# MarkJhonBao/InfantPoseEstimation_GaussianBias

Measured on AMD Instinct MI355X. Metric: images/sec (train fwd+bwd) HRFormer-S 256x192, higher is better.
Workload: dtype bf16; 1 GPU; HRFormer-small + fusion head, 256x192 -> 64x48, K=17, train step fwd+bwd+AdamW, DropPath 0.1, BN train; global_batch=64, per_gpu_batch=64, parallelism=dp1, launch=hipGraph replay, branches on concurrent HIP streams

## Files before the change

### infantposeestimation_gaussianbias_amd/csrc/pk_block.hip

```cpp
#include "pk_common.h"

typedef __attribute__((ext_vector_type(8))) short bf16x8;
typedef __attribute__((ext_vector_type(4))) float f32x4;
typedef __attribute__((ext_vector_type(4))) short s16x4;
typedef __attribute__((ext_vector_type(4))) unsigned int u32x4;
typedef __attribute__((ext_vector_type(2))) unsigned int u32x2;

#define OOB_OFF 0x80000000u
#define MAKE_RSRC(ptr) __builtin_amdgcn_make_buffer_rsrc(const_cast<uint16_t*>(ptr), 0, 0x7ffffff0, 0x00020000)
#define LOG2E_F 1.44269504088896340736f
#define MFMA(a, b, c) __builtin_amdgcn_mfma_f32_16x16x32_bf16(a, b, c, 0, 0, 0)
#define MFMA16(a, b, c) __builtin_amdgcn_mfma_f32_16x16x16bf16_1k(a, b, c, 0, 0, 0)
#define LO4(v) __builtin_shufflevector(v, v, 0, 1, 2, 3)
#define HI4(v) __builtin_shufflevector(v, v, 4, 5, 6, 7)
#define LDS_FENCE() asm volatile("s_waitcnt lgkmcnt(0)" ::: "memory")

struct MlpArgs {
    const uint16_t* x;
    const uint16_t* dy;
    uint16_t* out;
    const float *gamma, *beta, *b1, *b2;
    const float* scale;
    const uint16_t* w1;
    const uint16_t* w2;
    const uint16_t* w1t;
    const uint16_t* w2t;
    float* part;
    int M, rows_per_sample;
    float eps;
};

__device__ __forceinline__ int hid(int t, int i) { return 32 * (t >> 1) + 8 * (i >> 2) + 4 * (t & 1) + (i & 3); }
__device__ __forceinline__ float blo(uint32_t u) { return __uint_as_float(u << 16); }
__device__ __forceinline__ float bhi(uint32_t u) { return __uint_as_float(u & 0xffff0000u); }
__device__ __forceinline__ bf16x8 pack2(const f32x4 a, const f32x4 b) {
    const u32x4 v = {pack_bf16x2(a[0], a[1]), pack_bf16x2(a[2], a[3]), pack_bf16x2(b[0], b[1]), pack_bf16x2(b[2], b[3])};
    return __builtin_bit_cast(bf16x8, v);
}
__device__ __forceinline__ f32x4 unpack4(const u32x2 v) { return (f32x4){blo(v[0]), bhi(v[0]), blo(v[1]), bhi(v[1])}; }
__device__ __forceinline__ u32x2 pack4(const f32x4 v) { return (u32x2){pack_bf16x2(v[0], v[1]), pack_bf16x2(v[2], v[3])}; }
__device__ __forceinline__ float sum8(const bf16x8 f) {
    const u32x4 v = __builtin_bit_cast(u32x4, f);
    return ((blo(v[0]) + bhi(v[0])) + (blo(v[1]) + bhi(v[1]))) + ((blo(v[2]) + bhi(v[2])) + (blo(v[3]) + bhi(v[3])));
}
__device__ __forceinline__ bf16x8 tr_frag32(const uint16_t* tile, int pitch, int col0, int lane) {
    const int g = lane >> 4, i = lane & 15;
    const uint16_t* a0 = tile + (4 * g + (i >> 2)) * pitch + col0 + 4 * (i & 3);
    const s16x4 lo = __builtin_amdgcn_ds_read_tr16_b64_v4i16((__attribute__((address_space(3))) s16x4*)a0);
    const s16x4 hi = __builtin_amdgcn_ds_read_tr16_b64_v4i16((__attribute__((address_space(3))) s16x4*)(a0 + 16 * pitch));
    return (bf16x8){lo[0], lo[1], lo[2], lo[3], hi[0], hi[1], hi[2], hi[3]};
}

template <typename RowFn, typename K0Fn>
__device__ __forceinline__ void stage_frags(u32x4* dst, const uint16_t* __restrict__ src, int nfrag, int ld, RowFn row, K0Fn k0) {
    for (int idx = threadIdx.x; idx < nfrag * 64; idx += blockDim.x) {
        const int f = idx >> 6, l = idx & 63;
        dst[idx] = *reinterpret_cast<const u32x4*>(src + (size_t)row(f, l & 15) * ld + k0(f) + 8 * (l >> 4));
    }
}
#define LDS_FRAG(base, f, lane) __builtin_bit_cast(bf16x8, (base)[(f) * 64 + (lane)])
template <bool OPAQUE>
__device__ __forceinline__ int opaque_lane(int lane) {
    if (OPAQUE) asm volatile("" : "+v"(lane));
    return lane;
}

template <int NK>
__device__ __forceinline__ void ln_row(const u32x4 (&xr)[NK], const float (&gam)[NK][8], const float (&bet)[NK][8], float inv_c, float eps,
                                       bf16x8 (&vf)[NK], float& mean, float& rstd) {
    float v[NK][8];
    float s = 0.f;
#pragma unroll
    for (int k = 0; k < NK; ++k)
#pragma unroll
        for (int j = 0; j < 4; ++j) {
            v[k][2 * j] = blo(xr[k][j]);
            v[k][2 * j + 1] = bhi(xr[k][j]);
            s += v[k][2 * j] + v[k][2 * j + 1];
        }
    s = xor16_sum(s);
    s = xor32_sum(s);
    mean = s * inv_c;
    float q = 0.f;
#pragma unroll
    for (int k = 0; k < NK; ++k)
#pragma unroll
        for (int j = 0; j < 8; ++j) {
            v[k][j] -= mean;
            q += v[k][j] * v[k][j];
        }
    q = xor16_sum(q);
    q = xor32_sum(q);
    rstd = rsqrtf(q * inv_c + eps);
#pragma unroll
    for (int k = 0; k < NK; ++k) {
        u32x4 o;
#pragma unroll
        for (int j = 0; j < 4; ++j)
            o[j] = pack_bf16x2(v[k][2 * j] * rstd * gam[k][2 * j] + bet[k][2 * j], v[k][2 * j + 1] * rstd * gam[k][2 * j + 1] + bet[k][2 * j + 1]);
        vf[k] = __builtin_bit_cast(bf16x8, o);
    }
}
template <int NK>
__device__ __forceinline__ void scale_rows(const u32x4 (&r)[NK], float sc, bf16x8 (&f)[NK]) {
#pragma unroll
    for (int k = 0; k < NK; ++k) {
        u32x4 o;
#pragma unroll
        for (int j = 0; j < 4; ++j) o[j] = pack_bf16x2(blo(r[k][j]) * sc, bhi(r[k][j]) * sc);
        f[k] = __builtin_bit_cast(bf16x8, o);
    }
}

template <int C>
__global__ void __launch_bounds__(256) k_mlp_fwd(MlpArgs p) {
    constexpr int HD = 4 * C, NK = C / 32, NT = HD / 16, NS = HD / 32, NCT = C / 16, RT = 2;
    __shared__ __attribute__((aligned(16))) u32x4 sW1[NT * NK * 64];
    __shared__ __attribute__((aligned(16))) u32x4 sW2[NCT * NS * 64];
    __shared__ __attribute__((aligned(16))) float sB1[HD];
    const int tid = threadIdx.x, lane_ = tid & 63, wave = tid >> 6, i16 = lane_ & 15, g = lane_ >> 4;
    stage_frags(sW1, p.w1, NT * NK, C, [](int f, int i) { return hid(f / NK, i); }, [](int f) { return 32 * (f % NK); });
    stage_frags(sW2, p.w2, NCT * NS, HD, [](int f, int i) { return 16 * (f / NS) + i; }, [](int f) { return 32 * (f % NS); });
    for (int i = tid; i < HD; i += 256) sB1[i] = p.b1[i];
    float gam[NK][8], bet[NK][8];
#pragma unroll
    for (int k = 0; k < NK; ++k)
#pragma unroll
        for (int j = 0; j < 8; ++j) {
            gam[k][j] = p.gamma[32 * k + 8 * g + j];
            bet[k][j] = p.beta[32 * k + 8 * g + j];
        }
    f32x4 b2v[NCT];
#pragma unroll
    for (int ct = 0; ct < NCT; ++ct) b2v[ct] = *reinterpret_cast<const f32x4*>(p.b2 + 16 * ct + 4 * g);
    __syncthreads();
    const auto rx = MAKE_RSRC(p.x);
    const auto ro = MAKE_RSRC(p.out);
    const int ngroups = (p.M + 16 * RT - 1) / (16 * RT);
    const float inv_c = 1.f / (float)C;
    const f32x4 zero = {0.f, 0.f, 0.f, 0.f};
    for (int grp = blockIdx.x * 4 + wave; grp < ngroups; grp += gridDim.x * 4) {
        const int lane = opaque_lane<C != 32>(lane_);
        u32x4 xr[RT][NK];
        u32x2 xo[RT][NCT];
        unsigned rbase[RT];
        float sc[RT];
#pragma unroll
        for (int rt = 0; rt < RT; ++rt) {
            const int row = grp * 16 * RT + 16 * rt + i16;
            const bool ok = row < p.M;
            rbase[rt] = ok ? (unsigned)row * (unsigned)(C * 2) : OOB_OFF;
#pragma unroll
            for (int k = 0; k < NK; ++k) xr[rt][k] = __builtin_amdgcn_raw_buffer_load_b128(rx, ok ? rbase[rt] + (32 * k + 8 * g) * 2 : OOB_OFF, 0, 0);
#pragma unroll
            for (int ct = 0; ct < NCT; ++ct) xo[rt][ct] = __builtin_amdgcn_raw_buffer_load_b64(rx, ok ? rbase[rt] + (16 * ct + 4 * g) * 2 : OOB_OFF, 0, 0);
            sc[rt] = (p.scale && ok) ? p.scale[row / p.rows_per_sample] : 1.f;
        }
        bf16x8 vf[RT][NK];
#pragma unroll
        for (int rt = 0; rt < RT; ++rt) {
            float mean, rstd;
            ln_row<NK>(xr[rt], gam, bet, inv_c, p.eps, vf[rt], mean, rstd);
        }
        f32x4 y[RT][NCT];
#pragma unroll
        for (int rt = 0; rt < RT; ++rt)
#pragma unroll
            for (int ct = 0; ct < NCT; ++ct) y[rt][ct] = zero;
#pragma unroll
        for (int s = 0; s < NS; ++s) {
            f32x4 h[RT][2];
#pragma unroll
            for (int u = 0; u < 2; ++u) {
                const int t = 2 * s + u;
                const f32x4 bias = *reinterpret_cast<const f32x4*>(&sB1[32 * s + 8 * g + 4 * u]);
#pragma unroll
                for (int rt = 0; rt < RT; ++rt) h[rt][u] = bias;
#pragma unroll
                for (int k = 0; k < NK; ++k) {
                    const bf16x8 a = LDS_FRAG(sW1, t * NK + k, lane);
#pragma unroll
                    for (int rt = 0; rt < RT; ++rt) h[rt][u] = MFMA(a, vf[rt][k], h[rt][u]);
                }
#pragma unroll
                for (int rt = 0; rt < RT; ++rt) h[rt][u] = gelu_erf(h[rt][u]);
            }
            bf16x8 hf[RT];
#pragma unroll
            for (int rt = 0; rt < RT; ++rt) hf[rt] = pack2(h[rt][0], h[rt][1]);
#pragma unroll
            for (int ct = 0; ct < NCT; ++ct) {
                const bf16x8 a = LDS_FRAG(sW2, ct * NS + s, lane);
#pragma unroll
                for (int rt = 0; rt < RT; ++rt) y[rt][ct] = MFMA(a, hf[rt], y[rt][ct]);
            }
        }
#pragma unroll
        for (int rt = 0; rt < RT; ++rt)
#pragma unroll
            for (int ct = 0; ct < NCT; ++ct) {
                const f32x4 o = (y[rt][ct] + b2v[ct]) * sc[rt] + unpack4(xo[rt][ct]);
                __builtin_amdgcn_raw_buffer_store_b64(pack4(o), ro, rbase[rt] == OOB_OFF ? OOB_OFF : rbase[rt] + (16 * ct + 4 * g) * 2, 0, 0);
            }
    }
}

template <int NK, int NCT, int WAVES, bool RESIDENT>
__global__ void __launch_bounds__(64 * WAVES) k_mlp_fwd_w(MlpArgs p, int C, int c_real, int HD) {
    constexpr int RT = 2, NF = 2 * NK + NCT, NLD = (NF + WAVES - 1) / WAVES;
    extern __shared__ __attribute__((aligned(16))) unsigned char smem_w[];
    const int NS = HD >> 5, n_slots = RESIDENT ? NS : 2;
    u32x4* ring = reinterpret_cast<u32x4*>(smem_w);
    float* sB1 = reinterpret_cast<float*>(smem_w + n_slots * NF * 1024);
    const int tid = threadIdx.x, lane = tid & 63, wave = tid >> 6, i16 = lane & 15, g = lane >> 4;
    const auto rw1 = MAKE_RSRC(p.w1), rw2 = MAKE_RSRC(p.w2);
    unsigned soff[NLD], sstep[NLD];
#pragma unroll
    for (int j = 0; j < NLD; ++j) {
        const int f = wave + WAVES * j;
        if (f < 2 * NK) {
            const int u = f / NK, k = f - u * NK, col = 32 * k + 8 * g;
            soff[j] = col < C ? (unsigned)((hid(u, i16) * C + col) * 2) : OOB_OFF;
            sstep[j] = 64u * (unsigned)C;
        } else if (f < NF) {
            const int ct = f - 2 * NK;
            soff[j] = (unsigned)(((16 * ct + i16) * HD + 8 * g) * 2);
            sstep[j] = 64u;
        } else {
            soff[j] = OOB_OFF;
            sstep[j] = 0u;
        }
    }
    u32x4 st[NLD];
    auto load_slice = [&](int s) {
#pragma unroll
        for (int j = 0; j < NLD; ++j) {
            const int f = wave + WAVES * j;
            st[j] = f < 2 * NK ? __builtin_amdgcn_raw_buffer_load_b128(rw1, soff[j] + sstep[j] * (unsigned)s, 0, 0)
                               : __builtin_amdgcn_raw_buffer_load_b128(rw2, soff[j] + sstep[j] * (unsigned)s, 0, 0);
        }
    };
    auto write_slice = [&](int slot) {
#pragma unroll
        for (int j = 0; j < NLD; ++j) {
            const int f = wave + WAVES * j;
            if (f < NF) ring[(slot * NF + f) * 64 + lane] = st[j];
        }
    };
    load_slice(0);
    for (int i = tid; i < HD; i += 64 * WAVES) sB1[i] = p.b1[i];
    if (RESIDENT) {
        for (int s = 0; s < NS; ++s) {
            write_slice(s);
            if (s + 1 < NS) load_slice(s + 1);
        }
        __syncthreads();
    }
    const auto rx = MAKE_RSRC(p.x);
    const auto ro = MAKE_RSRC(p.out);
    const auto rgam = __builtin_amdgcn_make_buffer_rsrc(const_cast<float*>(p.gamma), 0, C * 4, 0x00020000);
    const auto rbet = __builtin_amdgcn_make_buffer_rsrc(const_cast<float*>(p.beta), 0, C * 4, 0x00020000);
    const auto rb2 = __builtin_amdgcn_make_buffer_rsrc(const_cast<float*>(p.b2), 0, C * 4, 0x00020000);
    const float inv_c = 1.f / (float)c_real, n_pad = (float)(32 * NK - c_real);
    const f32x4 zero = {0.f, 0.f, 0.f, 0.f};
    const int ngroups = (p.M + 16 * RT - 1) / (16 * RT);
    auto process = [&](const int grp) {
        unsigned rbase[RT];
        float sc[RT];
        bf16x8 vf[RT][NK];
#pragma unroll
        for (int rt = 0; rt < RT; ++rt) {
            const int row = grp * 16 * RT + 16 * rt + i16;
            const bool ok = row < p.M;
            rbase[rt] = ok ? (unsigned)row * (unsigned)(C * 2) : OOB_OFF;
            sc[rt] = (p.scale && ok) ? p.scale[row / p.rows_per_sample] : 1.f;
            u32x4 xr[NK];
#pragma unroll
            for (int k = 0; k < NK; ++k) xr[k] = __builtin_amdgcn_raw_buffer_load_b128(rx, (ok && 32 * k + 8 * g < C) ? rbase[rt] + (32 * k + 8 * g) * 2 : OOB_OFF, 0, 0);
            float v[NK][8];
            float sm = 0.f;
#pragma unroll
            for (int k = 0; k < NK; ++k)
#pragma unroll
                for (int j = 0; j < 4; ++j) {
                    v[k][2 * j] = blo(xr[k][j]);
                    v[k][2 * j + 1] = bhi(xr[k][j]);
                    sm += v[k][2 * j] + v[k][2 * j + 1];
                }
            sm = xor16_sum(sm);
            sm = xor32_sum(sm);
            const float mean = sm * inv_c;
            float q = 0.f;
#pragma unroll
            for (int k = 0; k < NK; ++k)
#pragma unroll
                for (int j = 0; j < 8; ++j) {
                    v[k][j] -= mean;
                    q += v[k][j] * v[k][j];
                }
            q = xor16_sum(q);
            q = xor32_sum(q);
            const float rstd = rsqrtf(fmaxf(q - n_pad * mean * mean, 0.f) * inv_c + p.eps);
#pragma unroll
            for (int k = 0; k < NK; ++k) {
                const f32x4 g0 = __builtin_bit_cast(f32x4, __builtin_amdgcn_raw_buffer_load_b128(rgam, (32 * k + 8 * g) * 4, 0, 0));
                const f32x4 g1 = __builtin_bit_cast(f32x4, __builtin_amdgcn_raw_buffer_load_b128(rgam, (32 * k + 8 * g + 4) * 4, 0, 0));
                const f32x4 b0 = __builtin_bit_cast(f32x4, __builtin_amdgcn_raw_buffer_load_b128(rbet, (32 * k + 8 * g) * 4, 0, 0));
                const f32x4 b1 = __builtin_bit_cast(f32x4, __builtin_amdgcn_raw_buffer_load_b128(rbet, (32 * k + 8 * g + 4) * 4, 0, 0));
                u32x4 o;
                o[0] = pack_bf16x2(v[k][0] * rstd * g0[0] + b0[0], v[k][1] * rstd * g0[1] + b0[1]);
                o[1] = pack_bf16x2(v[k][2] * rstd * g0[2] + b0[2], v[k][3] * rstd * g0[3] + b0[3]);
                o[2] = pack_bf16x2(v[k][4] * rstd * g1[0] + b1[0], v[k][5] * rstd * g1[1] + b1[1]);
                o[3] = pack_bf16x2(v[k][6] * rstd * g1[2] + b1[2], v[k][7] * rstd * g1[3] + b1[3]);
                vf[rt][k] = __builtin_bit_cast(bf16x8, o);
            }
        }
        if (!RESIDENT) {
            write_slice(0);
            if (NS > 1) load_slice(1);
        }
        f32x4 y[RT][NCT];
#pragma unroll
        for (int rt = 0; rt < RT; ++rt)
#pragma unroll
            for (int ct = 0; ct < NCT; ++ct) y[rt][ct] = zero;
#pragma unroll 1
        for (int s = 0; s < NS; ++s) {
            if (!RESIDENT) {
                __syncthreads();
                if (s + 1 < NS) write_slice((s + 1) & 1);
                if (s + 2 < NS) load_slice(s + 2);
            }
            const u32x4* fr = ring + (RESIDENT ? s : (s & 1)) * NF * 64;
            f32x4 h[RT][2];
#pragma unroll
            for (int u = 0; u < 2; ++u) {
                const f32x4 bias = *reinterpret_cast<const f32x4*>(&sB1[32 * s + 8 * g + 4 * u]);
#pragma unroll
                for (int rt = 0; rt < RT; ++rt) h[rt][u] = bias;
            }
#pragma unroll
            for (int k = 0; k < NK; ++k)
#pragma unroll
                for (int u = 0; u < 2; ++u) {
                    const bf16x8 a = LDS_FRAG(fr, u * NK + k, lane);
#pragma unroll
                    for (int rt = 0; rt < RT; ++rt) h[rt][u] = MFMA(a, vf[rt][k], h[rt][u]);
                }
            bf16x8 hf[RT];
#pragma unroll
            for (int rt = 0; rt < RT; ++rt) {
                hf[rt] = pack2(gelu_erf_poly(h[rt][0]), gelu_erf_poly(h[rt][1]));
            }
#pragma unroll
            for (int ct = 0; ct < NCT; ++ct) {
                const bf16x8 a = LDS_FRAG(fr, 2 * NK + ct, lane);
#pragma unroll
                for (int rt = 0; rt < RT; ++rt) y[rt][ct] = MFMA(a, hf[rt], y[rt][ct]);
            }
        }
#pragma unroll
        for (int rt = 0; rt < RT; ++rt)
#pragma unroll
            for (int ct = 0; ct < NCT; ++ct) {
                const unsigned off = rbase[rt] == OOB_OFF ? OOB_OFF : rbase[rt] + (16 * ct + 4 * g) * 2;
                const u32x2 xo = __builtin_amdgcn_raw_buffer_load_b64(rx, off, 0, 0);
                const f32x4 b2v = __builtin_bit_cast(f32x4, __builtin_amdgcn_raw_buffer_load_b128(rb2, (16 * ct + 4 * g) * 4, 0, 0));
                const f32x4 o = (y[rt][ct] + b2v) * sc[rt] + unpack4(xo);
                __builtin_amdgcn_raw_buffer_store_b64(pack4(o), ro, off, 0, 0);
            }
    };
    if (RESIDENT) {
        for (int grp = blockIdx.x * WAVES + wave; grp < ngroups; grp += gridDim.x * WAVES) process(grp);
    } else {
        process(blockIdx.x * WAVES + wave);
    }
}

template <int C>
__global__ void __launch_bounds__(256) k_mlp_bwd_dx(MlpArgs p) {
    constexpr int HD = 4 * C, NK = C / 32, NT = HD / 16, NS = HD / 32, NCT = C / 16, RT = 2;
    __shared__ __attribute__((aligned(16))) u32x4 sW1[NT * NK * 64];
    __shared__ __attribute__((aligned(16))) u32x4 sW2T[NT * NK * 64];
    __shared__ __attribute__((aligned(16))) u32x4 sW1T[NCT * NS * 64];
    __shared__ __attribute__((aligned(16))) float sB1[HD];
    __shared__ float sRed[4][2][C];
    const int tid = threadIdx.x, lane_ = tid & 63, wave = tid >> 6, i16 = lane_ & 15, g = lane_ >> 4;
    stage_frags(sW1, p.w1, NT * NK, C, [](int f, int i) { return hid(f / NK, i); }, [](int f) { return 32 * (f % NK); });
    stage_frags(sW2T, p.w2t, NT * NK, C, [](int f, int i) { return hid(f / NK, i); }, [](int f) { return 32 * (f % NK); });
    stage_frags(sW1T, p.w1t, NCT * NS, HD, [](int f, int i) { return 16 * (f / NS) + i; }, [](int f) { return 32 * (f % NS); });
    for (int i = tid; i < HD; i += 256) sB1[i] = p.b1[i];
    float gam[NK][8], bet[NK][8];
#pragma unroll
    for (int k = 0; k < NK; ++k)
#pragma unroll
        for (int j = 0; j < 8; ++j) {
            gam[k][j] = p.gamma[32 * k + 8 * g + j];
            bet[k][j] = p.beta[32 * k + 8 * g + j];
        }
    f32x4 gamA[NCT], dgam[NCT], dbet[NCT];
    const f32x4 zero = {0.f, 0.f, 0.f, 0.f};
#pragma unroll
    for (int ct = 0; ct < NCT; ++ct) {
        gamA[ct] = *reinterpret_cast<const f32x4*>(p.gamma + 16 * ct + 4 * g);
        dgam[ct] = dbet[ct] = zero;
    }
    __syncthreads();
    const auto rx = MAKE_RSRC(p.x);
    const auto rg = MAKE_RSRC(p.dy);
    const auto ro = MAKE_RSRC(p.out);
    const int ngroups = (p.M + 16 * RT - 1) / (16 * RT);
    const float inv_c = 1.f / (float)C;
    for (int grp = blockIdx.x * 4 + wave; grp < ngroups; grp += gridDim.x * 4) {
        const int lane = opaque_lane<true>(lane_);
        u32x4 xr[RT][NK], dyr[RT][NK];
        u32x2 xo[RT][NCT], dyo[RT][NCT];
        unsigned rbase[RT];
        float sc[RT];
#pragma unroll
        for (int rt = 0; rt < RT; ++rt) {
            const int row = grp * 16 * RT + 16 * rt + i16;
            const bool ok = row < p.M;
            rbase[rt] = ok ? (unsigned)row * (unsigned)(C * 2) : OOB_OFF;
#pragma unroll
            for (int k = 0; k < NK; ++k) {
                const unsigned off = ok ? rbase[rt] + (32 * k + 8 * g) * 2 : OOB_OFF;
                xr[rt][k] = __builtin_amdgcn_raw_buffer_load_b128(rx, off, 0, 0);
                dyr[rt][k] = __builtin_amdgcn_raw_buffer_load_b128(rg, off, 0, 0);
            }
#pragma unroll
            for (int ct = 0; ct < NCT; ++ct) {
                const unsigned off = ok ? rbase[rt] + (16 * ct + 4 * g) * 2 : OOB_OFF;
                xo[rt][ct] = __builtin_amdgcn_raw_buffer_load_b64(rx, off, 0, 0);
                dyo[rt][ct] = __builtin_amdgcn_raw_buffer_load_b64(rg, off, 0, 0);
            }
            sc[rt] = (p.scale && ok) ? p.scale[row / p.rows_per_sample] : 1.f;
        }
        bf16x8 vf[RT][NK], gf[RT][NK];
        float mean[RT], rstd[RT];
#pragma unroll
        for (int rt = 0; rt < RT; ++rt) {
            ln_row<NK>(xr[rt], gam, bet, inv_c, p.eps, vf[rt], mean[rt], rstd[rt]);
            scale_rows<NK>(dyr[rt], sc[rt], gf[rt]);
        }
        f32x4 dv[RT][NCT];
#pragma unroll
        for (int rt = 0; rt < RT; ++rt)
#pragma unroll
            for (int ct = 0; ct < NCT; ++ct) dv[rt][ct] = zero;
#pragma unroll
        for (int s = 0; s < NS; ++s) {
            f32x4 dz[RT][2];
#pragma unroll
            for (int u = 0; u < 2; ++u) {
                const int t = 2 * s + u;
                const f32x4 bias = *reinterpret_cast<const f32x4*>(&sB1[32 * s + 8 * g + 4 * u]);
                f32x4 z[RT], dh[RT];
#pragma unroll
                for (int rt = 0; rt < RT; ++rt) {
                    z[rt] = bias;
                    dh[rt] = zero;
                }
#pragma unroll
                for (int k = 0; k < NK; ++k) {
                    const bf16x8 a1 = LDS_FRAG(sW1, t * NK + k, lane), a2 = LDS_FRAG(sW2T, t * NK + k, lane);
#pragma unroll
                    for (int rt = 0; rt < RT; ++rt) {
                        z[rt] = MFMA(a1, vf[rt][k], z[rt]);
                        dh[rt] = MFMA(a2, gf[rt][k], dh[rt]);
                    }
                }
#pragma unroll
                for (int rt = 0; rt < RT; ++rt) dz[rt][u] = dh[rt] * gelu_grad(z[rt]);
            }
            bf16x8 dzf[RT];
#pragma unroll
            for (int rt = 0; rt < RT; ++rt) dzf[rt] = pack2(dz[rt][0], dz[rt][1]);
#pragma unroll
            for (int ct = 0; ct < NCT; ++ct) {
                const bf16x8 a = LDS_FRAG(sW1T, ct * NS + s, lane);
#pragma unroll
                for (int rt = 0; rt < RT; ++rt) dv[rt][ct] = MFMA(a, dzf[rt], dv[rt][ct]);
            }
        }
#pragma unroll
        for (int rt = 0; rt < RT; ++rt) {
            f32x4 xh[NCT];
            float s1 = 0.f, s2 = 0.f;
#pragma unroll
            for (int ct = 0; ct < NCT; ++ct) {
                xh[ct] = (unpack4(xo[rt][ct]) - mean[rt]) * rstd[rt];
#pragma unroll
                for (int r = 0; r < 4; ++r) {
                    const float gh = dv[rt][ct][r] * gamA[ct][r];
                    s1 += gh;
                    s2 += gh * xh[ct][r];
                }
                dgam[ct] += dv[rt][ct] * xh[ct];
                dbet[ct] += dv[rt][ct];
            }
            s1 = xor16_sum(s1);
            s1 = xor32_sum(s1);
            s2 = xor16_sum(s2);
            s2 = xor32_sum(s2);
            const float m1 = s1 * inv_c, m2 = s2 * inv_c;
#pragma unroll
            for (int ct = 0; ct < NCT; ++ct) {
                const f32x4 o = (dv[rt][ct] * gamA[ct] - m1 - xh[ct] * m2) * rstd[rt] + unpack4(dyo[rt][ct]);
                __builtin_amdgcn_raw_buffer_store_b64(pack4(o), ro, rbase[rt] == OOB_OFF ? OOB_OFF : rbase[rt] + (16 * ct + 4 * g) * 2, 0, 0);
            }
        }
    }
#pragma unroll
    for (int ct = 0; ct < NCT; ++ct)
#pragma unroll
        for (int r = 0; r < 4; ++r) {
            float a = dgam[ct][r], b = dbet[ct][r];
            a = lanes_sum<16>(a);
            b = lanes_sum<16>(b);
            if (i16 == 0) {
                sRed[wave][0][16 * ct + 4 * g + r] = a;
                sRed[wave][1][16 * ct + 4 * g + r] = b;
            }
        }
    __syncthreads();
    if (tid < 2 * C) {
        const int which = tid / C, c = tid - which * C;
        p.part[(size_t)blockIdx.x * 2 * C + tid] = ((sRed[0][which][c] + sRed[1][which][c]) + sRed[2][which][c]) + sRed[3][which][c];
    }
}

template <int C, int HS>
__global__ void __launch_bounds__(256) k_mlp_bwd_dw(MlpArgs p) {
    constexpr int NK = C / 32, NTS = HS / 16, NSP = HS / 32, NCT = C / 16, RT = 2;
    constexpr int PV = C + 8, PH = 40;
    constexpr int TILE_HALFS = 2 * 32 * PV + 2 * 32 * PH;
    constexpr int SLAB = 2 * HS * C + HS + C;
    constexpr int SCRATCH_BYTES = (4 * TILE_HALFS * 2 > SLAB * 4) ? 4 * TILE_HALFS * 2 : SLAB * 4;
    __shared__ __attribute__((aligned(16))) u32x4 sW1[NTS * NK * 64];
    __shared__ __attribute__((aligned(16))) u32x4 sW2T[NTS * NK * 64];
    __shared__ __attribute__((aligned(16))) float sB1[HS];
    __shared__ __attribute__((aligned(16))) unsigned char sScratch[SCRATCH_BYTES];
    const int tid = threadIdx.x, lane_ = tid & 63, wave = tid >> 6, i16 = lane_ & 15, g = lane_ >> 4;
    const int h0 = blockIdx.y * HS;
    stage_frags(sW1, p.w1 + (size_t)h0 * C, NTS * NK, C, [](int f, int i) { return 16 * (f / NK) + i; }, [](int f) { return 32 * (f % NK); });
    stage_frags(sW2T, p.w2t + (size_t)h0 * C, NTS * NK, C, [](int f, int i) { return 16 * (f / NK) + i; }, [](int f) { return 32 * (f % NK); });
    for (int i = tid; i < HS; i += 256) sB1[i] = p.b1[h0 + i];
    uint16_t* tV = reinterpret_cast<uint16_t*>(sScratch) + wave * TILE_HALFS;
    uint16_t* tG = tV + 32 * PV;
    uint16_t* tH = tG + 32 * PV;
    uint16_t* tD = tH + 32 * PH;
    float gam[NK][8], bet[NK][8];
#pragma unroll
    for (int k = 0; k < NK; ++k)
#pragma unroll
        for (int j = 0; j < 8; ++j) {
            gam[k][j] = p.gamma[32 * k + 8 * g + j];
            bet[k][j] = p.beta[32 * k + 8 * g + j];
        }
    const f32x4 zero = {0.f, 0.f, 0.f, 0.f};
    f32x4 dW1[NTS][NCT], dW2[NCT][NTS];
    float db1[NTS], db2[NCT];
#pragma unroll
    for (int t = 0; t < NTS; ++t) {
        db1[t] = 0.f;
#pragma unroll
        for (int ct = 0; ct < NCT; ++ct) dW1[t][ct] = dW2[ct][t] = zero;
    }
#pragma unroll
    for (int ct = 0; ct < NCT; ++ct) db2[ct] = 0.f;
    __syncthreads();
    const auto rx = MAKE_RSRC(p.x);
    const auto rg = MAKE_RSRC(p.dy);
    const int ngroups = (p.M + 16 * RT - 1) / (16 * RT);
    const float inv_c = 1.f / (float)C;
    for (int grp = blockIdx.x * 4 + wave; grp < ngroups; grp += gridDim.x * 4) {
        const int lane = opaque_lane<true>(lane_);
        u32x4 xr[RT][NK], dyr[RT][NK];
        float sc[RT];
#pragma unroll
        for (int rt = 0; rt < RT; ++rt) {
            const int row = grp * 16 * RT + 16 * rt + i16;
            const bool ok = row < p.M;
#pragma unroll
            for (int k = 0; k < NK; ++k) {
                const unsigned off = ok ? (unsigned)row * (unsigned)(C * 2) + (32 * k + 8 * g) * 2 : OOB_OFF;
                xr[rt][k] = __builtin_amdgcn_raw_buffer_load_b128(rx, off, 0, 0);
                dyr[rt][k] = __builtin_amdgcn_raw_buffer_load_b128(rg, off, 0, 0);
            }
            sc[rt] = (p.scale && ok) ? p.scale[row / p.rows_per_sample] : 1.f;
        }
        bf16x8 vf[RT][NK], gf[RT][NK];
#pragma unroll
        for (int rt = 0; rt < RT; ++rt) {
            float mean, rstd;
            ln_row<NK>(xr[rt], gam, bet, inv_c, p.eps, vf[rt], mean, rstd);
            scale_rows<NK>(dyr[rt], sc[rt], gf[rt]);
#pragma unroll
            for (int k = 0; k < NK; ++k) {
                *reinterpret_cast<bf16x8*>(tV + (16 * rt + i16) * PV + 32 * k + 8 * g) = vf[rt][k];
                *reinterpret_cast<bf16x8*>(tG + (16 * rt + i16) * PV + 32 * k + 8 * g) = gf[rt][k];
            }
        }
        LDS_FENCE();
        bf16x8 vT[NCT], gT[NCT];
#pragma unroll
        for (int ct = 0; ct < NCT; ++ct) {
            vT[ct] = tr_frag32(tV, PV, 16 * ct, lane);
            gT[ct] = tr_frag32(tG, PV, 16 * ct, lane);
            db2[ct] += sum8(gT[ct]);
        }
#pragma unroll
        for (int sp = 0; sp < NSP; ++sp) {
#pragma unroll
            for (int u = 0; u < 2; ++u) {
                const int t = 2 * sp + u;
                const f32x4 bias = *reinterpret_cast<const f32x4*>(&sB1[16 * t + 4 * g]);
                f32x4 z[RT], dh[RT];
#pragma unroll
                for (int rt = 0; rt < RT; ++rt) {
                    z[rt] = bias;
                    dh[rt] = zero;
                }
#pragma unroll
                for (int k = 0; k < NK; ++k) {
                    const bf16x8 a1 = LDS_FRAG(sW1, t * NK + k, lane), a2 = LDS_FRAG(sW2T, t * NK + k, lane);
#pragma unroll
                    for (int rt = 0; rt < RT; ++rt) {
                        z[rt] = MFMA(a1, vf[rt][k], z[rt]);
                        dh[rt] = MFMA(a2, gf[rt][k], dh[rt]);
                    }
                }
#pragma unroll
                for (int rt = 0; rt < RT; ++rt) {
                    f32x4 hh, dz;
                    gelu_both(z[rt], hh, dz);
                    dz *= dh[rt];
                    *reinterpret_cast<u32x2*>(tH + (16 * rt + i16) * PH + 16 * u + 4 * g) = pack4(hh);
                    *reinterpret_cast<u32x2*>(tD + (16 * rt + i16) * PH + 16 * u + 4 * g) = pack4(dz);
                }
            }
            LDS_FENCE();
#pragma unroll
            for (int u = 0; u < 2; ++u) {
                const int t = 2 * sp + u;
                const bf16x8 hT = tr_frag32(tH, PH, 16 * u, lane), dT = tr_frag32(tD, PH, 16 * u, lane);
                db1[t] += sum8(dT);
#pragma unroll
                for (int ct = 0; ct < NCT; ++ct) {
                    dW2[ct][t] = MFMA(gT[ct], hT, dW2[ct][t]);
                    dW1[t][ct] = MFMA(dT, vT[ct], dW1[t][ct]);
                }
            }
            LDS_FENCE();
        }
    }
    float* slab = reinterpret_cast<float*>(sScratch);
#pragma unroll 1
    for (int w = 0; w < 4; ++w) {
        __syncthreads();
        if (wave == w) {
#pragma unroll
            for (int t = 0; t < NTS; ++t) {
#pragma unroll
                for (int ct = 0; ct < NCT; ++ct)
#pragma unroll
                    for (int r = 0; r < 4; ++r) {
                        float* a = slab + (16 * t + 4 * g + r) * C + 16 * ct + i16;
                        float* b = slab + HS * C + (16 * ct + 4 * g + r) * HS + 16 * t + i16;
                        *a = (w ? *a : 0.f) + dW1[t][ct][r];
                        *b = (w ? *b : 0.f) + dW2[ct][t][r];
                    }
                float v = db1[t];
                v = xor16_sum(v);
                v = xor32_sum(v);
                if (g == 0) {
                    float* a = slab + 2 * HS * C + 16 * t + i16;
                    *a = (w ? *a : 0.f) + v;
                }
            }
#pragma unroll
            for (int ct = 0; ct < NCT; ++ct) {
                float v = db2[ct];
                v = xor16_sum(v);
                v = xor32_sum(v);
                if (g == 0) {
                    float* a = slab + 2 * HS * C + HS + 16 * ct + i16;
                    *a = (w ? *a : 0.f) + v;
                }
            }
        }
    }
    __syncthreads();
    float* dst = p.part + ((size_t)blockIdx.y * gridDim.x + blockIdx.x) * SLAB;
    for (int i = tid * 4; i < SLAB; i += 1024) *reinterpret_cast<f32x4*>(dst + i) = *reinterpret_cast<const f32x4*>(slab + i);
}

struct AttnArgs {
    const uint16_t* x;
    const uint16_t* dy;
    uint16_t* out;
    const int32_t* rowmap;
    const float *gamma, *beta, *table, *bqkv, *bproj, *scale;
    const uint16_t *wqkv, *wproj;
    const uint16_t *wqkv_t, *wproj_t;
    uint16_t* o_save;
    float* lse;
    uint16_t* dqkv;
    uint16_t* u_save;
    float* part;
    int n_windows, windows_per_sample;
    float eps, softmax_scale;
};
#define AT_N 49
__device__ __forceinline__ int rel_a7(int t) { return 13 * (t / 7) + t % 7; }

template <int C>
__global__ void __launch_bounds__(256) k_attn_fwd(AttnArgs p) {
    constexpr int HEADS = C / 32, NK = C / 32, NCT = C / 16;
    __shared__ __attribute__((aligned(16))) u32x4 sWqkv[HEADS * 6 * NK * 64];
    __shared__ __attribute__((aligned(16))) u32x4 sWp[NCT * HEADS * 64];
    __shared__ __attribute__((aligned(16))) float sBqkv[3 * C];
    __shared__ float sBias[HEADS][176];
    const int tid = threadIdx.x, lane_ = tid & 63, wave = tid >> 6, g_ = lane_ >> 4;
    stage_frags(sWqkv, p.wqkv, HEADS * 6 * NK, C,
                [](int f, int i) {
                    const int k_ = f % NK, r = f / NK, et = r & 1, part = (r >> 1) % 3, h = r / 6;
                    (void)k_;
                    return part * C + 32 * h + (part == 2 ? hid(et, i) : 16 * et + i);
                },
                [](int f) { return 32 * (f % NK); });
    stage_frags(sWp, p.wproj, NCT * HEADS, C, [](int f, int i) { return 16 * (f / HEADS) + i; }, [](int f) { return 32 * (f % HEADS); });
    for (int i = tid; i < 3 * C; i += 256) sBqkv[i] = p.bqkv[i];
    for (int i = tid; i < HEADS * 169; i += 256) sBias[i / 169][i % 169] = p.table[(i % 169) * HEADS + i / 169];
    float gam[NK][8], bet[NK][8];
#pragma unroll
    for (int k = 0; k < NK; ++k)
#pragma unroll
        for (int j = 0; j < 8; ++j) {
            gam[k][j] = p.gamma[32 * k + 8 * g_ + j];
            bet[k][j] = p.beta[32 * k + 8 * g_ + j];
        }
    f32x4 bpv[NCT];
#pragma unroll
    for (int ct = 0; ct < NCT; ++ct) bpv[ct] = *reinterpret_cast<const f32x4*>(p.bproj + 16 * ct + 4 * g_);
    int aj[4][4];
#pragma unroll
    for (int cj = 0; cj < 4; ++cj)
#pragma unroll
        for (int r = 0; r < 4; ++r) {
            const int j = 16 * cj + 4 * g_ + r;
            aj[cj][r] = j < AT_N ? 84 - rel_a7(j) : -1;
        }
    __syncthreads();
    const auto rx = MAKE_RSRC(p.x);
    const auto ro = MAKE_RSRC(p.out);
    const float inv_c = 1.f / (float)C;
    const f32x4 zero = {0.f, 0.f, 0.f, 0.f};
    for (int w = blockIdx.x * 4 + wave; w < p.n_windows; w += gridDim.x * 4) {
        const int lane = opaque_lane<true>(lane_), i16 = lane & 15, g = lane >> 4;
        int row[4];
        u32x4 xr[4][NK];
        u32x2 xo[4][NCT];
#pragma unroll
        for (int t = 0; t < 4; ++t) {
            const int n = 16 * t + i16;
            row[t] = n < AT_N ? p.rowmap[w * AT_N + n] : -1;
        }
#pragma unroll
        for (int t = 0; t < 4; ++t) {
            const unsigned base = row[t] >= 0 ? (unsigned)row[t] * (unsigned)(C * 2) : OOB_OFF;
#pragma unroll
            for (int k = 0; k < NK; ++k) xr[t][k] = __builtin_amdgcn_raw_buffer_load_b128(rx, row[t] >= 0 ? base + (32 * k + 8 * g) * 2 : OOB_OFF, 0, 0);
#pragma unroll
            for (int ct = 0; ct < NCT; ++ct) xo[t][ct] = __builtin_amdgcn_raw_buffer_load_b64(rx, row[t] >= 0 ? base + (16 * ct + 4 * g) * 2 : OOB_OFF, 0, 0);
        }
        const float sc = p.scale ? p.scale[w / p.windows_per_sample] : 1.f;
        bf16x8 uf[4][NK];
#pragma unroll
        for (int t = 0; t < 4; ++t) {
            float mean, rstd;
            ln_row<NK>(xr[t], gam, bet, inv_c, p.eps, uf[t], mean, rstd);
            if (row[t] < 0) {
#pragma unroll
                for (int k = 0; k < NK; ++k) uf[t][k] = (bf16x8){0, 0, 0, 0, 0, 0, 0, 0};
            }
        }
        f32x4 accY[4][NCT];
#pragma unroll
        for (int t = 0; t < 4; ++t)
#pragma unroll
            for (int ct = 0; ct < NCT; ++ct) accY[t][ct] = zero;
#pragma unroll 1
        for (int h = 0; h < HEADS; ++h) {
            bf16x8 qf[4], kf[4], vt[2][2];
            {
                f32x4 va[4][2];
#pragma unroll
                for (int ce = 0; ce < 2; ++ce) {
                    const float bv = sBqkv[2 * C + 32 * h + hid(ce, i16)];
#pragma unroll
                    for (int t = 0; t < 4; ++t) va[t][ce] = (f32x4){bv, bv, bv, bv};
#pragma unroll
                    for (int k = 0; k < NK; ++k) {
                        const bf16x8 wv = LDS_FRAG(sWqkv, ((h * 3 + 2) * 2 + ce) * NK + k, lane);
#pragma unroll
                        for (int t = 0; t < 4; ++t) va[t][ce] = MFMA(uf[t][k], wv, va[t][ce]);
                    }
                }
#pragma unroll
                for (int s = 0; s < 2; ++s)
#pragma unroll
                    for (int ce = 0; ce < 2; ++ce) vt[s][ce] = pack2(va[2 * s][ce], va[2 * s + 1][ce]);
            }
            {
                f32x4 qa[4][2], ka[4][2];
#pragma unroll
                for (int et = 0; et < 2; ++et) {
                    const f32x4 bq = *reinterpret_cast<const f32x4*>(&sBqkv[32 * h + 16 * et + 4 * g]);
                    const f32x4 bk = *reinterpret_cast<const f32x4*>(&sBqkv[C + 32 * h + 16 * et + 4 * g]);
#pragma unroll
                    for (int t = 0; t < 4; ++t) {
                        qa[t][et] = bq;
                        ka[t][et] = bk;
                    }
#pragma unroll
                    for (int k = 0; k < NK; ++k) {
                        const bf16x8 wq = LDS_FRAG(sWqkv, ((h * 3 + 0) * 2 + et) * NK + k, lane);
                        const bf16x8 wk = LDS_FRAG(sWqkv, ((h * 3 + 1) * 2 + et) * NK + k, lane);
#pragma unroll
                        for (int t = 0; t < 4; ++t) {
                            qa[t][et] = MFMA(wq, uf[t][k], qa[t][et]);
                            ka[t][et] = MFMA(wk, uf[t][k], ka[t][et]);
                        }
                    }
                }
#pragma unroll
                for (int t = 0; t < 4; ++t) {
                    qf[t] = pack2(qa[t][0], qa[t][1]);
                    kf[t] = pack2(ka[t][0], ka[t][1]);
                }
            }
#pragma unroll
            for (int ci = 0; ci < 4; ++ci) {
                const int i = 16 * ci + i16;
                const int ai = rel_a7(i < AT_N ? i : 0);
                f32x4 st[4];
#pragma unroll
                for (int cj = 0; cj < 4; ++cj) st[cj] = MFMA(kf[cj], qf[ci], zero);
                float mx = -INFINITY;
#pragma unroll
                for (int cj = 0; cj < 4; ++cj)
#pragma unroll
                    for (int r = 0; r < 4; ++r) {
                        const float bv = sBias[h][ai + (aj[cj][r] >= 0 ? aj[cj][r] : 0)];
                        st[cj][r] = aj[cj][r] >= 0 ? st[cj][r] * p.softmax_scale + bv : -INFINITY;
                        mx = fmaxf(mx, st[cj][r]);
                    }
                mx = xor16_max(mx);
                mx = xor32_max(mx);
                float sum = 0.f;
#pragma unroll
                for (int cj = 0; cj < 4; ++cj)
#pragma unroll
                    for (int r = 0; r < 4; ++r) {
                        st[cj][r] = __expf(st[cj][r] - mx);
                        sum += st[cj][r];
                    }
                sum = xor16_sum(sum);
                sum = xor32_sum(sum);
                const float inv = 1.f / sum;
                if (g == 0 && i < AT_N && p.lse) p.lse[((size_t)w * HEADS + h) * AT_N + i] = mx + __logf(sum);
                const bf16x8 p0 = pack2(st[0] * inv, st[1] * inv), p1 = pack2(st[2] * inv, st[3] * inv);
                f32x4 o[2];
#pragma unroll
                for (int ce = 0; ce < 2; ++ce) {
                    o[ce] = MFMA(vt[0][ce], p0, zero);
                    o[ce] = MFMA(vt[1][ce], p1, o[ce]);
                    if (p.o_save && i < AT_N)
                        *reinterpret_cast<u32x2*>(p.o_save + ((size_t)w * AT_N + i) * C + 32 * h + 8 * g + 4 * ce) = pack4(o[ce]);
                }
                const bf16x8 of = pack2(o[0], o[1]);
#pragma unroll
                for (int nt = 0; nt < NCT; ++nt) accY[ci][nt] = MFMA(LDS_FRAG(sWp, nt * HEADS + h, lane), of, accY[ci][nt]);
            }
        }
#pragma unroll
        for (int t = 0; t < 4; ++t)
#pragma unroll
            for (int ct = 0; ct < NCT; ++ct) {
                const f32x4 v = (accY[t][ct] + bpv[ct]) * sc + unpack4(xo[t][ct]);
                __builtin_amdgcn_raw_buffer_store_b64(pack4(v), ro, row[t] >= 0 ? (unsigned)row[t] * (unsigned)(C * 2) + (16 * ct + 4 * g) * 2 : OOB_OFF, 0, 0);
            }
    }
}

template <int NK, int NCT, int HEADS, int WAVES>
__global__ void __launch_bounds__(64 * WAVES) k_attn_fwd_w(AttnArgs p, int C, int c_real) {
    constexpr int NT_ = 64 * WAVES;
    constexpr int ET = 3, HDP = 40;
    constexpr int F_QK = 2 * ET * NK, F_V = ET * NK, F_P = NCT, F_HEAD = F_QK + F_V + F_P;
    extern __shared__ __attribute__((aligned(16))) unsigned char smem_a[];
    u32x4* sW = reinterpret_cast<u32x4*>(smem_a);
    u32x2* sP2 = reinterpret_cast<u32x2*>(smem_a + HEADS * F_HEAD * 1024);
    float* sBqkv = reinterpret_cast<float*>(smem_a + HEADS * (F_HEAD * 1024 + NCT * 512));
    f32x4* sBias = reinterpret_cast<f32x4*>(sBqkv + 3 * HEADS * HDP);
    const int tid = threadIdx.x, lane_ = tid & 63, wave = tid >> 6, g_ = lane_ >> 4;
    for (int idx = tid; idx < HEADS * F_HEAD * 64; idx += NT_) {
        const int f = idx >> 6, l = idx & 63, i = l & 15, gg = l >> 4, h = f / F_HEAD, fl = f - h * F_HEAD;
        u32x4 v = {0u, 0u, 0u, 0u};
        if (fl < F_QK + F_V) {
            int row, k;
            if (fl < F_QK) {
                const int part = fl / (ET * NK), r = fl - part * ET * NK, et = r / NK;
                k = r - et * NK;
                const int e = 16 * et + i;
                row = e < HDP ? part * C + HDP * h + e : -1;
            } else {
                const int r = fl - F_QK, ce = r / NK;
                k = r - ce * NK;
                const int e = ce < 2 ? hid(ce, i) : (i < 8 ? 32 + i : HDP);
                row = e < HDP ? 2 * C + HDP * h + e : -1;
            }
            const int col = 32 * k + 8 * gg;
            if (row >= 0 && col < C) v = *reinterpret_cast<const u32x4*>(p.wqkv + (size_t)row * C + col);
        } else {
            const int nt = fl - F_QK - F_V;
            v = *reinterpret_cast<const u32x4*>(p.wproj + (size_t)(16 * nt + i) * C + HDP * h + 8 * gg);
        }
        sW[idx] = v;
    }
    for (int idx = tid; idx < HEADS * NCT * 64; idx += NT_) {
        const int f = idx >> 6, l = idx & 63, i = l & 15, gg = l >> 4, h = f / NCT, nt = f - h * NCT;
        u32x2 v = {0u, 0u};
        if (gg < 2) v = *reinterpret_cast<const u32x2*>(p.wproj + (size_t)(16 * nt + i) * C + HDP * h + 32 + 4 * gg);
        sP2[idx] = v;
    }
    for (int i = tid; i < 3 * C; i += NT_) sBqkv[i] = p.bqkv[i];
    for (int idx = tid; idx < HEADS * 16 * 64; idx += NT_) {
        const int l = idx & 63, tile = (idx >> 6) & 15, h = idx >> 10, ci = tile >> 2, cj = tile & 3;
        const int i = 16 * ci + (l & 15), ai = rel_a7(i < AT_N ? i : 0);
        f32x4 v;
#pragma unroll
        for (int r = 0; r < 4; ++r) {
            const int j = 16 * cj + 4 * (l >> 4) + r;
            v[r] = j < AT_N ? p.table[(ai - rel_a7(j) + 84) * HEADS + h] * 1.44269504088896340736f : -INFINITY;
        }
        sBias[idx] = v;
    }
    __syncthreads();
    const auto rx = MAKE_RSRC(p.x);
    const auto ro = MAKE_RSRC(p.out);
    const auto rgam = __builtin_amdgcn_make_buffer_rsrc(const_cast<float*>(p.gamma), 0, C * 4, 0x00020000);
    const auto rbet = __builtin_amdgcn_make_buffer_rsrc(const_cast<float*>(p.beta), 0, C * 4, 0x00020000);
    const auto rbp = __builtin_amdgcn_make_buffer_rsrc(const_cast<float*>(p.bproj), 0, C * 4, 0x00020000);
    const float inv_c = 1.f / (float)c_real, n_pad = (float)(32 * NK - c_real);
    const f32x4 zero = {0.f, 0.f, 0.f, 0.f};
    const float qscale = p.softmax_scale * 1.44269504088896340736f;
    for (int w = blockIdx.x * WAVES + wave; w < p.n_windows; w += gridDim.x * WAVES) {
        const int lane = opaque_lane<true>(lane_), i16 = lane & 15, g = lane >> 4;
        int row[4];
#pragma unroll
        for (int t = 0; t < 4; ++t) {
            const int n = 16 * t + i16;
            row[t] = n < AT_N ? p.rowmap[w * AT_N + n] : -1;
        }
        const float sc = p.scale ? p.scale[w / p.windows_per_sample] : 1.f;
        bf16x8 uf[4][NK];
#pragma unroll
        for (int t = 0; t < 4; ++t) {
            const unsigned base = row[t] >= 0 ? (unsigned)row[t] * (unsigned)(C * 2) : OOB_OFF;
            u32x4 xr[NK];
#pragma unroll
            for (int k = 0; k < NK; ++k)
                xr[k] = __builtin_amdgcn_raw_buffer_load_b128(rx, (row[t] >= 0 && 32 * k + 8 * g < C) ? base + (32 * k + 8 * g) * 2 : OOB_OFF, 0, 0);
            float v[NK][8];
            float sm = 0.f;
#pragma unroll
            for (int k = 0; k < NK; ++k)
#pragma unroll
                for (int j = 0; j < 4; ++j) {
                    v[k][2 * j] = blo(xr[k][j]);
                    v[k][2 * j + 1] = bhi(xr[k][j]);
                    sm += v[k][2 * j] + v[k][2 * j + 1];
                }
            sm = xor16_sum(sm);
            sm = xor32_sum(sm);
            const float mean = sm * inv_c;
            float qv = 0.f;
#pragma unroll
            for (int k = 0; k < NK; ++k)
#pragma unroll
                for (int j = 0; j < 8; ++j) {
                    v[k][j] -= mean;
                    qv += v[k][j] * v[k][j];
                }
            qv = xor16_sum(qv);
            qv = xor32_sum(qv);
            const float rstd = rsqrtf(fmaxf(qv - n_pad * mean * mean, 0.f) * inv_c + p.eps);
#pragma unroll
            for (int k = 0; k < NK; ++k) {
                const f32x4 g0 = __builtin_bit_cast(f32x4, __builtin_amdgcn_raw_buffer_load_b128(rgam, (32 * k + 8 * g) * 4, 0, 0));
                const f32x4 g1 = __builtin_bit_cast(f32x4, __builtin_amdgcn_raw_buffer_load_b128(rgam, (32 * k + 8 * g + 4) * 4, 0, 0));
                const f32x4 b0 = __builtin_bit_cast(f32x4, __builtin_amdgcn_raw_buffer_load_b128(rbet, (32 * k + 8 * g) * 4, 0, 0));
                const f32x4 b1 = __builtin_bit_cast(f32x4, __builtin_amdgcn_raw_buffer_load_b128(rbet, (32 * k + 8 * g + 4) * 4, 0, 0));
                u32x4 o;
                o[0] = pack_bf16x2(v[k][0] * rstd * g0[0] + b0[0], v[k][1] * rstd * g0[1] + b0[1]);
                o[1] = pack_bf16x2(v[k][2] * rstd * g0[2] + b0[2], v[k][3] * rstd * g0[3] + b0[3]);
                o[2] = pack_bf16x2(v[k][4] * rstd * g1[0] + b1[0], v[k][5] * rstd * g1[1] + b1[1]);
                o[3] = pack_bf16x2(v[k][6] * rstd * g1[2] + b1[2], v[k][7] * rstd * g1[3] + b1[3]);
                uf[t][k] = row[t] >= 0 ? __builtin_bit_cast(bf16x8, o) : (bf16x8){0, 0, 0, 0, 0, 0, 0, 0};
            }
        }
        f32x4 accY[4][NCT];
#pragma unroll
        for (int t = 0; t < 4; ++t)
#pragma unroll
            for (int ct = 0; ct < NCT; ++ct) accY[t][ct] = zero;
#pragma unroll 1
        for (int h = 0; h < HEADS; ++h) {
            const u32x4* hw = sW + h * F_HEAD * 64;
            const float* hb = sBqkv + HDP * h;
            bf16x8 kf[4], vt[2][ET];
            s16x4 kf2[4];
            {
                f32x4 va[4][ET];
#pragma unroll
                for (int ce = 0; ce < ET; ++ce) {
                    const int e = ce < 2 ? hid(ce, i16) : (i16 < 8 ? 32 + i16 : -1);
                    const float bv = e >= 0 ? hb[2 * C + e] : 0.f;
#pragma unroll
                    for (int t = 0; t < 4; ++t) va[t][ce] = (f32x4){bv, bv, bv, bv};
#pragma unroll
                    for (int k = 0; k < NK; ++k) {
                        const bf16x8 wv = LDS_FRAG(hw, F_QK + ce * NK + k, lane);
#pragma unroll
                        for (int t = 0; t < 4; ++t) va[t][ce] = MFMA(uf[t][k], wv, va[t][ce]);
                    }
                }
#pragma unroll
                for (int s2 = 0; s2 < 2; ++s2)
#pragma unroll
                    for (int ce = 0; ce < ET; ++ce) vt[s2][ce] = pack2(va[2 * s2][ce], va[2 * s2 + 1][ce]);
            }
            {
                f32x4 ka[4][ET];
#pragma unroll
                for (int et = 0; et < ET; ++et) {
                    f32x4 bk = zero;
                    if (et < 2 || g < 2) bk = *reinterpret_cast<const f32x4*>(&hb[C + 16 * et + 4 * g]);
#pragma unroll
                    for (int t = 0; t < 4; ++t) ka[t][et] = bk;
#pragma unroll
                    for (int k = 0; k < NK; ++k) {
                        const bf16x8 wk = LDS_FRAG(hw, (ET + et) * NK + k, lane);
#pragma unroll
                        for (int t = 0; t < 4; ++t) ka[t][et] = MFMA(wk, uf[t][k], ka[t][et]);
                    }
                }
#pragma unroll
                for (int t = 0; t < 4; ++t) {
                    kf[t] = pack2(ka[t][0], ka[t][1]);
                    kf2[t] = __builtin_bit_cast(s16x4, pack4(ka[t][2]));
                }
            }
#pragma unroll
            for (int ci = 0; ci < 4; ++ci) {
                bf16x8 qf;
                s16x4 qf2;
                {
                    f32x4 qa[ET];
#pragma unroll
                    for (int et = 0; et < ET; ++et) {
                        qa[et] = zero;
                        if (et < 2 || g < 2) qa[et] = *reinterpret_cast<const f32x4*>(&hb[16 * et + 4 * g]);
#pragma unroll
                        for (int k = 0; k < NK; ++k) qa[et] = MFMA(LDS_FRAG(hw, et * NK + k, lane), uf[ci][k], qa[et]);
                    }
                    qf = pack2(qa[0], qa[1]);
                    qf2 = __builtin_bit_cast(s16x4, pack4(qa[2]));
                }
                f32x4 st[4];
#pragma unroll
                for (int cj = 0; cj < 4; ++cj) {
                    st[cj] = MFMA16(LO4(kf[cj]), LO4(qf), zero);
                    st[cj] = MFMA16(HI4(kf[cj]), HI4(qf), st[cj]);
                    st[cj] = MFMA16(kf2[cj], qf2, st[cj]);
                }
                float mx = -INFINITY;
#pragma unroll
                for (int cj = 0; cj < 4; ++cj) {
                    st[cj] = __builtin_elementwise_fma(st[cj], (f32x4)(qscale), sBias[((h * 4 + ci) * 4 + cj) * 64 + lane]);
                    mx = fmaxf(fmaxf(mx, fmaxf(st[cj][0], st[cj][1])), fmaxf(st[cj][2], st[cj][3]));
                }
                mx = xor16_max(mx);
                mx = xor32_max(mx);
                float sum = 0.f;
#pragma unroll
                for (int cj = 0; cj < 4; ++cj)
#pragma unroll
                    for (int r = 0; r < 4; ++r) {
                        st[cj][r] = __builtin_amdgcn_exp2f(st[cj][r] - mx);
                        sum += st[cj][r];
                    }
                sum = xor16_sum(sum);
                sum = xor32_sum(sum);
                const float inv = 1.f / sum;
                const bf16x8 p0 = pack2(st[0] * inv, st[1] * inv), p1 = pack2(st[2] * inv, st[3] * inv);
                f32x4 o[ET];
#pragma unroll
                for (int ce = 0; ce < ET; ++ce) {
                    o[ce] = MFMA(vt[0][ce], p0, zero);
                    o[ce] = MFMA(vt[1][ce], p1, o[ce]);
                }
                const bf16x8 of0 = pack2(o[0], o[1]);
                const s16x4 of1 = __builtin_bit_cast(s16x4, pack4(o[2]));
#pragma unroll
                for (int nt = 0; nt < NCT; ++nt) {
                    const bf16x8 wp = LDS_FRAG(hw, F_QK + F_V + nt, lane);
                    accY[ci][nt] = MFMA16(LO4(wp), LO4(of0), accY[ci][nt]);
                    accY[ci][nt] = MFMA16(HI4(wp), HI4(of0), accY[ci][nt]);
                    accY[ci][nt] = MFMA16(__builtin_bit_cast(s16x4, sP2[(h * NCT + nt) * 64 + lane]), of1, accY[ci][nt]);
                }
            }
        }
#pragma unroll
        for (int t = 0; t < 4; ++t)
#pragma unroll
            for (int ct = 0; ct < NCT; ++ct) {
                const unsigned off = row[t] >= 0 ? (unsigned)row[t] * (unsigned)(C * 2) + (16 * ct + 4 * g) * 2 : OOB_OFF;
                const u32x2 xo = __builtin_amdgcn_raw_buffer_load_b64(rx, off, 0, 0);
                const f32x4 bp = __builtin_bit_cast(f32x4, __builtin_amdgcn_raw_buffer_load_b128(rbp, (16 * ct + 4 * g) * 4, 0, 0));
                const f32x4 v = (accY[t][ct] + bp) * sc + unpack4(xo);
                __builtin_amdgcn_raw_buffer_store_b64(pack4(v), ro, off, 0, 0);
            }
    }
}

template <int C>
__global__ void __launch_bounds__(256, 2) k_attn_bwd(AttnArgs p, float* __restrict__ part_ln, float* __restrict__ part_rpb) {
    constexpr int HEADS = C / 32, NK = C / 32, NCT = C / 16, NKQ = 3 * C / 32;
    constexpr int F_A = 6 * NK, F_B = 4 * NK;
    __shared__ __attribute__((aligned(16))) u32x4 sWa[HEADS * F_A * 64];
    __shared__ __attribute__((aligned(16))) u32x4 sWb[HEADS * F_B * 64];
    __shared__ __attribute__((aligned(16))) u32x4 sPa[HEADS * 2 * NK * 64];
    __shared__ __attribute__((aligned(16))) u32x4 sPb[HEADS * 2 * NK * 64];
    __shared__ __attribute__((aligned(16))) u32x4 sWt[NCT * NKQ * 64];
    __shared__ __attribute__((aligned(16))) float sBqkv[3 * C];
    __shared__ __attribute__((aligned(16))) float sGam[C], sBet[C];
    __shared__ __attribute__((aligned(16))) int sA[64];
    __shared__ float sBias[HEADS][176];
    __shared__ __attribute__((aligned(16))) float sLse[4][64], sDelta[4][64];
    __shared__ float sMean[4][64], sRstd[4][64];
    __shared__ int sRow[4][64];
    __shared__ float sTab[4][HEADS][192];
    constexpr int FOLD_PAD = 296;
    __shared__ float sFoldBuf[FOLD_PAD + 4 * AT_N * AT_N + FOLD_PAD];
    float* const sFold0 = sFoldBuf + FOLD_PAD;
    __shared__ float sRed[4][2][C];
    const int tid = threadIdx.x, lane_ = tid & 63, wave = tid >> 6;
    stage_frags(sWa, p.wqkv, HEADS * F_A, C,
                [](int f, int i) { const int r = f / NK, et = r & 1, part = (r >> 1) % 3, h = r / 6; return part * C + 32 * h + 16 * et + i; },
                [](int f) { return 32 * (f % NK); });
    stage_frags(sWb, p.wqkv, HEADS * F_B, C,
                [](int f, int i) { const int r = f / NK, ce = r & 1, part = (r >> 1) & 1, h = r / 4; return part * C + 32 * h + hid(ce, i); },
                [](int f) { return 32 * (f % NK); });
    stage_frags(sPa, p.wproj_t, HEADS * 2 * NK, C, [](int f, int i) { const int r = f / NK; return 32 * (r >> 1) + 16 * (r & 1) + i; },
                [](int f) { return 32 * (f % NK); });
    stage_frags(sPb, p.wproj_t, HEADS * 2 * NK, C, [](int f, int i) { const int r = f / NK; return 32 * (r >> 1) + hid(r & 1, i); },
                [](int f) { return 32 * (f % NK); });
    stage_frags(sWt, p.wqkv_t, NCT * NKQ, 3 * C, [](int f, int i) { return 16 * (f / NKQ) + i; }, [](int f) { return 32 * (f % NKQ); });
    for (int i = tid; i < 3 * C; i += 256) sBqkv[i] = p.bqkv[i];
    for (int i = tid; i < C; i += 256) {
        sGam[i] = p.gamma[i];
        sBet[i] = p.beta[i];
    }
    if (tid < 64) sA[tid] = tid < AT_N ? rel_a7(tid) : -1;
    for (int i = tid; i < HEADS * 169; i += 256) sBias[i / 169][i % 169] = p.table[(i % 169) * HEADS + i / 169] * LOG2E_F;
    for (int i = tid; i < 4 * HEADS * 192; i += 256) (&sTab[0][0][0])[i] = 0.f;
    const f32x4 zero = {0.f, 0.f, 0.f, 0.f};
    f32x4 dgam[NCT], dbet[NCT];
#pragma unroll
    for (int ct = 0; ct < NCT; ++ct) dgam[ct] = dbet[ct] = zero;
    __syncthreads();
    const auto rx = MAKE_RSRC(p.x);
    const auto rg = MAKE_RSRC(p.dy);
    const auto ro = MAKE_RSRC(p.out);
    const auto rs = MAKE_RSRC(p.o_save);
    const float inv_c = 1.f / (float)C, scale = p.softmax_scale, scale2 = p.softmax_scale * LOG2E_F, inv_scale = 1.f / p.softmax_scale;
    for (int w = blockIdx.x * 4 + wave; w < p.n_windows; w += gridDim.x * 4) {
        const int lane = opaque_lane<true>(lane_), i16 = lane & 15, g = lane >> 4;
        int row[4];
        f32x4 du[4][NCT];
#pragma unroll
        for (int t = 0; t < 4; ++t)
#pragma unroll
            for (int ct = 0; ct < NCT; ++ct) du[t][ct] = zero;
        {
            u32x4 xr[4][NK], dyr[4][NK];
#pragma unroll
            for (int t = 0; t < 4; ++t) {
                const int n = 16 * t + i16;
                row[t] = n < AT_N ? p.rowmap[w * AT_N + n] : -1;
            }
#pragma unroll
            for (int t = 0; t < 4; ++t)
#pragma unroll
                for (int k = 0; k < NK; ++k) {
                    const unsigned off = row[t] >= 0 ? (unsigned)row[t] * (unsigned)(C * 2) + (32 * k + 8 * g) * 2 : OOB_OFF;
                    xr[t][k] = __builtin_amdgcn_raw_buffer_load_b128(rx, off, 0, 0);
                    dyr[t][k] = __builtin_amdgcn_raw_buffer_load_b128(rg, off, 0, 0);
                }
            const float sc = p.scale ? p.scale[w / p.windows_per_sample] : 1.f;
            bf16x8 uf[4][NK], gf[4][NK];
            {
                float gam[NK][8], bet[NK][8];
#pragma unroll
                for (int k = 0; k < NK; ++k) {
                    *reinterpret_cast<f32x4*>(&gam[k][0]) = *reinterpret_cast<const f32x4*>(&sGam[32 * k + 8 * g]);
                    *reinterpret_cast<f32x4*>(&gam[k][4]) = *reinterpret_cast<const f32x4*>(&sGam[32 * k + 8 * g + 4]);
                    *reinterpret_cast<f32x4*>(&bet[k][0]) = *reinterpret_cast<const f32x4*>(&sBet[32 * k + 8 * g]);
                    *reinterpret_cast<f32x4*>(&bet[k][4]) = *reinterpret_cast<const f32x4*>(&sBet[32 * k + 8 * g + 4]);
                }
#pragma unroll
                for (int t = 0; t < 4; ++t) {
                    float mean_t, rstd_t;
                    ln_row<NK>(xr[t], gam, bet, inv_c, p.eps, uf[t], mean_t, rstd_t);
                    if (g == 0) {
                        sMean[wave][16 * t + i16] = mean_t;
                        sRstd[wave][16 * t + i16] = rstd_t;
                        sRow[wave][16 * t + i16] = row[t];
                    }
                    scale_rows<NK>(dyr[t], sc, gf[t]);
                    if (row[t] < 0) {
#pragma unroll
                        for (int k = 0; k < NK; ++k) uf[t][k] = (bf16x8){0, 0, 0, 0, 0, 0, 0, 0};
                    }
                    if (16 * t + i16 < AT_N) {
#pragma unroll
                        for (int k = 0; k < NK; ++k)
                            *reinterpret_cast<bf16x8*>(p.u_save + ((size_t)w * AT_N + 16 * t + i16) * C + 32 * k + 8 * g) = uf[t][k];
                    }
                }
            }
            uint16_t* dq_base = p.dqkv + (size_t)w * AT_N * 3 * C;
#pragma unroll 1
            for (int h = 0; h < HEADS; ++h) {
                bf16x8 qf[4], kf[4], vf[4], dof[4];
                u32x2 osv[4][2];
                float lsv[4];
#pragma unroll
                for (int t = 0; t < 4; ++t) {
                    const int i = 16 * t + i16;
                    const unsigned ob = i < AT_N ? (unsigned)((w * AT_N + i) * C + 32 * h + 4 * g) * 2u : OOB_OFF;
                    osv[t][0] = __builtin_amdgcn_raw_buffer_load_b64(rs, ob, 0, 0);
                    osv[t][1] = __builtin_amdgcn_raw_buffer_load_b64(rs, i < AT_N ? ob + 32 : OOB_OFF, 0, 0);
                    lsv[t] = i < AT_N ? p.lse[((size_t)w * HEADS + h) * AT_N + i] : 0.f;
                }
#pragma unroll
                for (int t = 0; t < 4; ++t) {
                    f32x4 a[4][2];
#pragma unroll
                    for (int et = 0; et < 2; ++et) {
#pragma unroll
                        for (int part = 0; part < 3; ++part) a[part][et] = *reinterpret_cast<const f32x4*>(&sBqkv[part * C + 32 * h + 16 * et + 4 * g]);
                        a[3][et] = zero;
#pragma unroll
                        for (int k = 0; k < NK; ++k) {
#pragma unroll
                            for (int part = 0; part < 3; ++part)
                                a[part][et] = MFMA(LDS_FRAG(sWa, ((h * 3 + part) * 2 + et) * NK + k, lane), uf[t][k], a[part][et]);
                            a[3][et] = MFMA(LDS_FRAG(sPa, (h * 2 + et) * NK + k, lane), gf[t][k], a[3][et]);
                        }
                    }
                    qf[t] = pack2(a[0][0], a[0][1]);
                    kf[t] = pack2(a[1][0], a[1][1]);
                    vf[t] = pack2(a[2][0], a[2][1]);
                    dof[t] = pack2(a[3][0], a[3][1]);
                    const int i = 16 * t + i16;
                    const f32x4 o0 = unpack4(osv[t][0]), o1 = unpack4(osv[t][1]);
                    float de = 0.f;
#pragma unroll
                    for (int r = 0; r < 4; ++r) de += a[3][0][r] * o0[r] + a[3][1][r] * o1[r];
                    de = xor16_sum(de);
                    de = xor32_sum(de);
                    if (g == 0) {
                        sLse[wave][i] = -lsv[t] * inv_scale;
                        sDelta[wave][i] = -de;
                    }
                }
                bf16x8 Kt[2][2];
#pragma unroll
                for (int ce = 0; ce < 2; ++ce) {
                    f32x4 a[4];
                    const float bk = sBqkv[C + 32 * h + hid(ce, i16)];
#pragma unroll
                    for (int t = 0; t < 4; ++t) a[t] = (f32x4){bk, bk, bk, bk};
#pragma unroll
                    for (int k = 0; k < NK; ++k) {
                        const bf16x8 wk = LDS_FRAG(sWb, ((h * 2 + 1) * 2 + ce) * NK + k, lane);
#pragma unroll
                        for (int t = 0; t < 4; ++t) a[t] = MFMA(uf[t][k], wk, a[t]);
                    }
#pragma unroll
                    for (int s = 0; s < 2; ++s) Kt[s][ce] = pack2(a[2 * s], a[2 * s + 1]);
                }
                LDS_FENCE();
#pragma unroll
                for (int ci = 0; ci < 4; ++ci) {
                    const int i = 16 * ci + i16;
                    const bool iok = ci < 3 || i16 == 0;
                    const int ai = rel_a7(iok ? i : 0) + 84;
                    const float li = sLse[wave][i], di = sDelta[wave][i];
                    const f32x4 li4 = {li, li, li, li}, di4 = {di, di, di, di};
                    f32x4 dq[2] = {zero, zero};
#pragma unroll
                    for (int s = 0; s < 2; ++s) {
                        f32x4 ds[2];
#pragma unroll
                        for (int u = 0; u < 2; ++u) {
                            const int cj = 2 * s + u;
                            const f32x4 scr = MFMA(kf[cj], qf[ci], li4), dp = MFMA(vf[cj], dof[ci], di4);
                            const int4 aj = *reinterpret_cast<const int4*>(&sA[16 * cj + 4 * g]);
                            const int ajr[4] = {aj.x, aj.y, aj.z, aj.w};
#pragma unroll
                            for (int r = 0; r < 4; ++r) {
                                const bool jv = cj < 3 || (g == 0 && r == 0);
                                const int e = ai - (cj < 3 ? ajr[r] : max(ajr[r], 0));
                                const float ev = __builtin_amdgcn_exp2f(__builtin_fmaf(scr[r], scale2, sBias[h][e]));
                                const float pv = (iok && jv) ? ev : 0.f;
                                ds[u][r] = pv * dp[r];
                                if (iok && jv) sFold0[wave * (AT_N * AT_N) + i * AT_N + 16 * cj + 4 * g + r] = ds[u][r];
                            }
                        }
                        const bf16x8 df = pack2(ds[0], ds[1]);
#pragma unroll
                        for (int ce = 0; ce < 2; ++ce) dq[ce] = MFMA(Kt[s][ce], df, dq[ce]);
                    }
                    {
                        const u32x2 q0 = pack4(dq[0] * scale), q1 = pack4(dq[1] * scale);
                        const u32x4 qv = iok ? (u32x4){q0[0], q0[1], q1[0], q1[1]} : (u32x4){0u, 0u, 0u, 0u};
                        if (iok) *reinterpret_cast<u32x4*>(dq_base + (size_t)i * 3 * C + 32 * h + 8 * g) = qv;
#pragma unroll
                        for (int ct = 0; ct < NCT; ++ct)
                            du[ci][ct] = MFMA(LDS_FRAG(sWt, ct * NKQ + h, lane), __builtin_bit_cast(bf16x8, qv), du[ci][ct]);
                    }
                }
                {
                    LDS_FENCE();
                    for (int e = lane; e < 169; e += 64) {
                        const int dy_ = e / 13 - 6, dx_ = e % 13 - 6;
                        const int x0 = max(0, -dx_), x1 = min(7, 7 - dx_);
                        const int base = wave * (AT_N * AT_N) + (dy_ * 7 + dx_) * AT_N;
                        unsigned keep[7];
#pragma unroll
                        for (int xj = 0; xj < 7; ++xj) keep[xj] = (xj >= x0 && xj < x1) ? 0xffffffffu : 0u;
                        float acc = 0.f;
                        for (int yj = max(0, -dy_); yj < min(7, 7 - dy_); ++yj) {
#pragma unroll
                            for (int xj = 0; xj < 7; ++xj) {
                                const float v = sFold0[base + yj * (7 * AT_N + 7) + xj * (AT_N + 1)];
                                acc += __uint_as_float(__float_as_uint(v) & keep[xj]);
                            }
                        }
                        sTab[wave][h][e] += acc;
                    }
                    LDS_FENCE();
                }
                bf16x8 Qt[2][2], dOt[2][2];
#pragma unroll
                for (int ce = 0; ce < 2; ++ce) {
                    f32x4 a[2][4];
                    const float bq = sBqkv[32 * h + hid(ce, i16)];
#pragma unroll
                    for (int t = 0; t < 4; ++t) {
                        a[0][t] = (f32x4){bq, bq, bq, bq};
                        a[1][t] = zero;
                    }
#pragma unroll
                    for (int k = 0; k < NK; ++k) {
                        const bf16x8 wq = LDS_FRAG(sWb, ((h * 2 + 0) * 2 + ce) * NK + k, lane), wp = LDS_FRAG(sPb, (h * 2 + ce) * NK + k, lane);
#pragma unroll
                        for (int t = 0; t < 4; ++t) {
                            a[0][t] = MFMA(uf[t][k], wq, a[0][t]);
                            a[1][t] = MFMA(gf[t][k], wp, a[1][t]);
                        }
                    }
#pragma unroll
                    for (int s = 0; s < 2; ++s) {
                        Qt[s][ce] = pack2(a[0][2 * s], a[0][2 * s + 1]);
                        dOt[s][ce] = pack2(a[1][2 * s], a[1][2 * s + 1]);
                    }
                }
#pragma unroll
                for (int cj = 0; cj < 4; ++cj) {
                    const int j = 16 * cj + i16;
                    const bool jok = cj < 3 || i16 == 0;
                    const int ajn = 84 - rel_a7(jok ? j : 0);
                    f32x4 dv[2] = {zero, zero}, dk[2] = {zero, zero};
#pragma unroll
                    for (int s = 0; s < 2; ++s) {
                        f32x4 pp[2], ds[2];
#pragma unroll
                        for (int u = 0; u < 2; ++u) {
                            const int ci = 2 * s + u;
                            const f32x4 l4 = *reinterpret_cast<const f32x4*>(&sLse[wave][16 * ci + 4 * g]);
                            const f32x4 de4 = *reinterpret_cast<const f32x4*>(&sDelta[wave][16 * ci + 4 * g]);
                            const f32x4 scr = MFMA(qf[ci], kf[cj], l4), dp = MFMA(dof[ci], vf[cj], de4);
                            const int4 aq = *reinterpret_cast<const int4*>(&sA[16 * ci + 4 * g]);
                            const int aqr[4] = {aq.x, aq.y, aq.z, aq.w};
#pragma unroll
                            for (int r = 0; r < 4; ++r) {
                                const bool iv = ci < 3 || (g == 0 && r == 0);
                                const float ev = __builtin_amdgcn_exp2f(__builtin_fmaf(scr[r], scale2, sBias[h][(ci < 3 ? aqr[r] : max(aqr[r], 0)) + ajn]));
                                const float pv = (jok && iv) ? ev : 0.f;
                                pp[u][r] = pv;
                                ds[u][r] = pv * dp[r];
                            }
                        }
                        const bf16x8 pf = pack2(pp[0], pp[1]), df = pack2(ds[0], ds[1]);
#pragma unroll
                        for (int ce = 0; ce < 2; ++ce) {
                            dv[ce] = MFMA(dOt[s][ce], pf, dv[ce]);
                            dk[ce] = MFMA(Qt[s][ce], df, dk[ce]);
                        }
                    }
                    {
                        const u32x2 k0 = pack4(dk[0] * scale), k1 = pack4(dk[1] * scale), v0 = pack4(dv[0]), v1 = pack4(dv[1]);
                        const u32x4 kv = jok ? (u32x4){k0[0], k0[1], k1[0], k1[1]} : (u32x4){0u, 0u, 0u, 0u};
                        const u32x4 vv = jok ? (u32x4){v0[0], v0[1], v1[0], v1[1]} : (u32x4){0u, 0u, 0u, 0u};
                        if (jok) {
                            *reinterpret_cast<u32x4*>(dq_base + (size_t)j * 3 * C + C + 32 * h + 8 * g) = kv;
                            *reinterpret_cast<u32x4*>(dq_base + (size_t)j * 3 * C + 2 * C + 32 * h + 8 * g) = vv;
                        }
#pragma unroll
                        for (int ct = 0; ct < NCT; ++ct) {
                            du[cj][ct] = MFMA(LDS_FRAG(sWt, ct * NKQ + HEADS + h, lane), __builtin_bit_cast(bf16x8, kv), du[cj][ct]);
                            du[cj][ct] = MFMA(LDS_FRAG(sWt, ct * NKQ + 2 * HEADS + h, lane), __builtin_bit_cast(bf16x8, vv), du[cj][ct]);
                        }
                    }
                }
                LDS_FENCE();
            }
        }
        u32x2 xo4[4][NCT], dyo4[4][NCT];
        int row2[4];
#pragma unroll
        for (int t = 0; t < 4; ++t) row2[t] = sRow[wave][16 * t + i16];
#pragma unroll
        for (int t = 0; t < 4; ++t)
#pragma unroll
            for (int ct = 0; ct < NCT; ++ct) {
                const unsigned off = row2[t] >= 0 ? (unsigned)row2[t] * (unsigned)(C * 2) + (16 * ct + 4 * g) * 2 : OOB_OFF;
                xo4[t][ct] = __builtin_amdgcn_raw_buffer_load_b64(rx, off, 0, 0);
                dyo4[t][ct] = __builtin_amdgcn_raw_buffer_load_b64(rg, off, 0, 0);
            }
#pragma unroll
        for (int t = 0; t < 4; ++t) {
            const int rw = row2[t];
            const float mu = sMean[wave][16 * t + i16], rsd = sRstd[wave][16 * t + i16];
            const bool valid = rw >= 0;
            f32x4 xh[NCT], gamA[NCT];
            float s1 = 0.f, s2 = 0.f;
#pragma unroll
            for (int ct = 0; ct < NCT; ++ct) {
                gamA[ct] = *reinterpret_cast<const f32x4*>(&sGam[16 * ct + 4 * g]);
                xh[ct] = (unpack4(xo4[t][ct]) - mu) * rsd;
#pragma unroll
                for (int r = 0; r < 4; ++r) {
                    const float gh = du[t][ct][r] * gamA[ct][r];
                    s1 += gh;
                    s2 += gh * xh[ct][r];
                }
                if (valid) {
                    dgam[ct] += du[t][ct] * xh[ct];
                    dbet[ct] += du[t][ct];
                }
            }
            s1 = xor16_sum(s1);
            s1 = xor32_sum(s1);
            s2 = xor16_sum(s2);
            s2 = xor32_sum(s2);
            const float m1 = s1 * inv_c, m2 = s2 * inv_c;
#pragma unroll
            for (int ct = 0; ct < NCT; ++ct) {
                const f32x4 o = (du[t][ct] * gamA[ct] - m1 - xh[ct] * m2) * rsd + unpack4(dyo4[t][ct]);
                __builtin_amdgcn_raw_buffer_store_b64(pack4(o), ro, valid ? (unsigned)rw * (unsigned)(C * 2) + (16 * ct + 4 * g) * 2 : OOB_OFF, 0, 0);
            }
        }
    }
    const int i16 = lane_ & 15, g = lane_ >> 4;
#pragma unroll
    for (int ct = 0; ct < NCT; ++ct)
#pragma unroll
        for (int r = 0; r < 4; ++r) {
            float a = dgam[ct][r], b = dbet[ct][r];
            a = lanes_sum<16>(a);
            b = lanes_sum<16>(b);
            if (i16 == 0) {
                sRed[wave][0][16 * ct + 4 * g + r] = a;
                sRed[wave][1][16 * ct + 4 * g + r] = b;
            }
        }
    __syncthreads();
    for (int i = tid; i < 4 * HEADS * 169; i += 256) {
        const int wv = i / (HEADS * 169), r = i % (HEADS * 169);
        part_rpb[((size_t)blockIdx.x * 4 + wv) * HEADS * 169 + r] = sTab[wv][r / 169][r % 169];
    }
    if (tid < 2 * C) {
        const int which = tid / C, c = tid - which * C;
        part_ln[(size_t)blockIdx.x * 2 * C + tid] = ((sRed[0][which][c] + sRed[1][which][c]) + sRed[2][which][c]) + sRed[3][which][c];
    }
}

static inline int attn_blocks(int n_windows) {
    constexpr int cap = 256;
    const int need = (n_windows + 3) / 4;
    return need < cap ? (need < 1 ? 1 : need) : cap;
}
extern "C" int pk_attn_block_blocks(int n_windows) { return attn_blocks(n_windows); }
extern "C" int pk_attn_block_bwd(const void* dy, const void* x, const int32_t* rowmap, const float* gamma, const float* beta,
                                 const float* rel_table, const void* wqkv, const float* bqkv, const void* wqkv_t, const void* wproj_t,
                                 const float* row_scale, const void* o_saved, const float* lse, void* dx, void* dqkv, void* u_out,
                                 float* ln_partial, float* rpb_partial, int n_windows, int windows_per_sample, int heads, int C, float eps,
                                 void* stream) {
    PK_SUPPORTED((C == 32 || C == 64) && heads * 32 == C, "pk_attn_block_bwd: C=%d heads=%d (built for C = 32 / 64 with head_dim 32)", C, heads);
    PK_REQUIRE(dy && x && rowmap && gamma && beta && rel_table && wqkv && bqkv && wqkv_t && wproj_t && o_saved && lse && dx && dqkv && u_out &&
               ln_partial && rpb_partial && n_windows > 0, "pk_attn_block_bwd: null pointer");
    PK_REQUIRE(!row_scale || windows_per_sample > 0, "pk_attn_block_bwd: row_scale needs windows_per_sample");
    PK_REQUIRE(((((uintptr_t)x) | ((uintptr_t)dy) | ((uintptr_t)dx) | ((uintptr_t)wqkv) | ((uintptr_t)wqkv_t) | ((uintptr_t)wproj_t) |
                 ((uintptr_t)o_saved) | ((uintptr_t)dqkv) | ((uintptr_t)u_out) | ((uintptr_t)gamma)) & 15) == 0, "pk_attn_block_bwd: 16-byte alignment");
    PK_REQUIRE((int64_t)n_windows * AT_N * 3 * C < 0x3fffffffLL, "pk_attn_block_bwd: too large for 32-bit offsets");
    AttnArgs a{};
    a.x = (const uint16_t*)x; a.dy = (const uint16_t*)dy; a.out = (uint16_t*)dx; a.rowmap = rowmap; a.gamma = gamma; a.beta = beta;
    a.table = rel_table; a.bqkv = bqkv; a.scale = row_scale; a.wqkv = (const uint16_t*)wqkv; a.wqkv_t = (const uint16_t*)wqkv_t;
    a.wproj_t = (const uint16_t*)wproj_t; a.o_save = (uint16_t*)const_cast<void*>(o_saved); a.lse = const_cast<float*>(lse);
    a.dqkv = (uint16_t*)dqkv; a.u_save = (uint16_t*)u_out; a.n_windows = n_windows;
    a.windows_per_sample = windows_per_sample > 0 ? windows_per_sample : 1; a.eps = eps; a.softmax_scale = 1.f / sqrtf(32.f);
    const dim3 grid(attn_blocks(n_windows)), block(256);
    if (C == 32) hipLaunchKernelGGL(k_attn_bwd<32>, grid, block, 0, (hipStream_t)stream, a, ln_partial, rpb_partial);
    else hipLaunchKernelGGL(k_attn_bwd<64>, grid, block, 0, (hipStream_t)stream, a, ln_partial, rpb_partial);
    return pk_launch_status("pk_attn_block_bwd");
}
extern "C" int pk_attn_block_supported(int C, int heads) { return (C == 32 || C == 64) && heads * 32 == C; }
extern "C" int pk_attn_block_fwd(const void* x, const int32_t* rowmap, const float* gamma, const float* beta, const float* rel_table,
                                 const void* wqkv, const float* bqkv, const void* wproj, const float* bproj, const float* row_scale,
                                 void* y, void* o_save, float* lse, int n_windows, int windows_per_sample, int heads, int C, float eps,
                                 void* stream) {
    PK_SUPPORTED(pk_attn_block_supported(C, heads), "pk_attn_block_fwd: C=%d heads=%d (built for C = 32 / 64 with head_dim 32)", C, heads);
    PK_REQUIRE(x && rowmap && gamma && beta && rel_table && wqkv && bqkv && wproj && bproj && y && n_windows > 0, "pk_attn_block_fwd: null pointer");
    PK_REQUIRE(!row_scale || windows_per_sample > 0, "pk_attn_block_fwd: row_scale needs windows_per_sample");
    PK_REQUIRE(((((uintptr_t)x) | ((uintptr_t)y) | ((uintptr_t)wqkv) | ((uintptr_t)wproj) | ((uintptr_t)o_save) | ((uintptr_t)bproj)) & 15) == 0,
               "pk_attn_block_fwd: 16-byte alignment");
    PK_REQUIRE((int64_t)n_windows * AT_N * 3 * C < 0x3fffffffLL, "pk_attn_block_fwd: too large for 32-bit offsets");
    AttnArgs a{};
    a.x = (const uint16_t*)x; a.out = (uint16_t*)y; a.rowmap = rowmap; a.gamma = gamma; a.beta = beta; a.table = rel_table; a.bqkv = bqkv;
    a.bproj = bproj; a.scale = row_scale; a.wqkv = (const uint16_t*)wqkv; a.wproj = (const uint16_t*)wproj; a.o_save = (uint16_t*)o_save;
    a.lse = lse; a.n_windows = n_windows; a.windows_per_sample = windows_per_sample > 0 ? windows_per_sample : 1; a.eps = eps;
    a.softmax_scale = 1.f / sqrtf(32.f);
    const dim3 grid(attn_blocks(n_windows)), block(256);
    if (C == 32) hipLaunchKernelGGL(k_attn_fwd<32>, grid, block, 0, (hipStream_t)stream, a);
    else hipLaunchKernelGGL(k_attn_fwd<64>, grid, block, 0, (hipStream_t)stream, a);
    return pk_launch_status("pk_attn_block_fwd");
}

extern "C" int pk_attn_block_wide_supported(int C, int heads, int n_windows) {
    constexpr int min_win = 1024;
    if (!(C == 80 && heads == 2)) return 0;
    return n_windows <= 0 || n_windows >= min_win;
}
template <int NK, int NCT, int HEADS, int WAVES>
static int attn_wide_launch(const AttnArgs& a, int C, int c_real, hipStream_t st) {
    const int lds = HEADS * ((3 * 3 * NK + NCT) * 1024 + NCT * 512) + 3 * C * 4 + HEADS * 16 * 1024;
    static bool attr_set = false;
    if (!attr_set) {
        hipError_t e = hipFuncSetAttribute((const void*)k_attn_fwd_w<NK, NCT, HEADS, WAVES>, hipFuncAttributeMaxDynamicSharedMemorySize, lds);
        if (e != hipSuccess) {
            pk_set_error("pk_attn_block_wide_fwd: cannot raise the LDS limit: %s", hipGetErrorString(e));
            return (int)e;
        }
        attr_set = true;
    }
    constexpr int cap = 256;
    const int need = (a.n_windows + WAVES - 1) / WAVES;
    hipLaunchKernelGGL((k_attn_fwd_w<NK, NCT, HEADS, WAVES>), dim3(need < cap ? need : cap), dim3(64 * WAVES), lds, st, a, C, c_real);
    return pk_launch_status("pk_attn_block_wide_fwd");
}
extern "C" int pk_attn_block_wide_fwd(const void* x, const int32_t* rowmap, const float* gamma, const float* beta, const float* rel_table,
                                      const void* wqkv, const float* bqkv, const void* wproj, const float* bproj, const float* row_scale,
                                      void* y, int n_windows, int windows_per_sample, int heads, int C, int c_real, float softmax_scale,
                                      float eps, void* stream) {
    PK_SUPPORTED(pk_attn_block_wide_supported(C, heads, 0), "pk_attn_block_wide_fwd: C=%d heads=%d (built for C = 80 with 2 heads of 40)", C, heads);
    PK_REQUIRE(x && rowmap && gamma && beta && rel_table && wqkv && bqkv && wproj && bproj && y && n_windows > 0, "pk_attn_block_wide_fwd: null pointer");
    PK_REQUIRE(c_real > 0 && c_real <= C && softmax_scale > 0.f, "pk_attn_block_wide_fwd: c_real=%d / softmax_scale=%g", c_real, (double)softmax_scale);
    PK_REQUIRE(!row_scale || windows_per_sample > 0, "pk_attn_block_wide_fwd: row_scale needs windows_per_sample");
    PK_REQUIRE(((((uintptr_t)x) | ((uintptr_t)y) | ((uintptr_t)wqkv) | ((uintptr_t)wproj) | ((uintptr_t)gamma) | ((uintptr_t)beta) | ((uintptr_t)bproj)) & 15) == 0,
               "pk_attn_block_wide_fwd: 16-byte alignment");
    PK_REQUIRE((int64_t)n_windows * AT_N * 3 * C < 0x3fffffffLL, "pk_attn_block_wide_fwd: too large for 32-bit offsets");
    AttnArgs a{};
    a.x = (const uint16_t*)x; a.out = (uint16_t*)y; a.rowmap = rowmap; a.gamma = gamma; a.beta = beta; a.table = rel_table; a.bqkv = bqkv;
    a.bproj = bproj; a.scale = row_scale; a.wqkv = (const uint16_t*)wqkv; a.wproj = (const uint16_t*)wproj;
    a.n_windows = n_windows; a.windows_per_sample = windows_per_sample > 0 ? windows_per_sample : 1; a.eps = eps; a.softmax_scale = softmax_scale;
    return attn_wide_launch<3, 5, 2, 8>(a, C, c_real, (hipStream_t)stream);
}

static inline int mlp_hidden_slice(int C) {
    return C == 32 ? 64 : 32;
}
static inline int mlp_row_groups(int M) { return (M + 31) / 32; }
extern "C" int pk_ln_mlp_supported(int C) { return C == 32 || C == 64; }
extern "C" int pk_ln_mlp_hidden_slice(int C) { return mlp_hidden_slice(C); }
extern "C" int pk_ln_mlp_slab_floats(int C) {
    const int hs = mlp_hidden_slice(C);
    return 2 * hs * C + hs + C;
}
static inline int mlp_blocks(int M, int target) {
    const int need = (mlp_row_groups(M) + 3) / 4;
    return need < target ? (need < 1 ? 1 : need) : target;
}
constexpr int MLP_FWD_WGS = 512, MLP_DX_WGS = 512;
static inline int mlp_dw_target(int C) {
    return C == 32 ? 256 : 32;
}
extern "C" int pk_ln_mlp_dx_blocks(int M, int C) { return mlp_blocks(M, MLP_DX_WGS); }
extern "C" int pk_ln_mlp_dw_blocks(int M, int C) { return mlp_blocks(M, mlp_dw_target(C)); }

static int mlp_check(const char* who, const MlpArgs& a, int C) {
    PK_SUPPORTED(C == 32 || C == 64, "%s: C=%d (the fused MLP half is built for C = 32 / 64)", who, C);
    PK_REQUIRE(a.x && a.gamma && a.beta && a.b1 && a.M > 0, "%s: null pointer / bad size", who);
    PK_REQUIRE(!a.scale || a.rows_per_sample > 0, "%s: scale needs rows_per_sample", who);
    PK_REQUIRE((int64_t)a.M * C < 0x3fffffffLL, "%s: tensor too large for 32-bit byte offsets", who);
    PK_REQUIRE(((((uintptr_t)a.x) | ((uintptr_t)a.dy) | ((uintptr_t)a.out) | ((uintptr_t)a.w1) | ((uintptr_t)a.w2) | ((uintptr_t)a.w1t) |
                 ((uintptr_t)a.w2t) | ((uintptr_t)a.gamma) | ((uintptr_t)a.b2) | ((uintptr_t)a.part)) & 15) == 0, "%s: 16-byte alignment", who);
    return PK_OK;
}

extern "C" int pk_ln_mlp_fwd(const void* x, const float* gamma, const float* beta, const void* w1, const float* b1, const void* w2,
                             const float* b2, const float* row_scale, void* y, int M, int C, int rows_per_sample, float eps, void* stream) {
    MlpArgs a{};
    a.x = (const uint16_t*)x; a.out = (uint16_t*)y; a.gamma = gamma; a.beta = beta; a.b1 = b1; a.b2 = b2; a.scale = row_scale;
    a.w1 = (const uint16_t*)w1; a.w2 = (const uint16_t*)w2; a.M = M; a.rows_per_sample = rows_per_sample > 0 ? rows_per_sample : 1; a.eps = eps;
    int rc = mlp_check("pk_ln_mlp_fwd", a, C);
    if (rc) return rc;
    PK_REQUIRE(w1 && w2 && b2 && y, "pk_ln_mlp_fwd: null pointer");
    const dim3 grid(mlp_blocks(M, MLP_FWD_WGS)), block(256);
    if (C == 32) hipLaunchKernelGGL(k_mlp_fwd<32>, grid, block, 0, (hipStream_t)stream, a);
    else hipLaunchKernelGGL(k_mlp_fwd<64>, grid, block, 0, (hipStream_t)stream, a);
    return pk_launch_status("pk_ln_mlp_fwd");
}

static int pk_cu_count_block() {
    static int n = 0;
    if (!n) {
        int dev = 0;
        hipDeviceProp_t prop;
        n = (hipGetDevice(&dev) == hipSuccess && hipGetDeviceProperties(&prop, dev) == hipSuccess && prop.multiProcessorCount > 0) ? prop.multiProcessorCount : 256;
    }
    return n;
}
extern "C" int pk_ln_mlp_wide_supported(int C, int hidden, int M) {
    constexpr int min_wgs = 160;
    if (!((C == 80 || C == 128 || C == 160 || C == 256 || C == 320) && hidden > 0 && hidden % 32 == 0 && hidden <= 2048)) return 0;
    const int per_wg = C >= 256 ? 128 : 256;
    return M <= 0 || (M + per_wg - 1) / per_wg >= min_wgs;
}
template <int NK, int NCT, int WAVES>
static int mlp_wide_launch(const MlpArgs& a, int C, int c_real, int HD, hipStream_t st) {
    constexpr int NF = 2 * NK + NCT;
    const int NS = HD / 32, lds_res = NS * NF * 1024 + HD * 4;
    const bool resident = lds_res <= 150 * 1024;
    const int lds = resident ? lds_res : 2 * NF * 1024 + HD * 4;
    static bool attr_set = false;
    if (!attr_set) {
        hipError_t e = hipFuncSetAttribute((const void*)k_mlp_fwd_w<NK, NCT, WAVES, true>, hipFuncAttributeMaxDynamicSharedMemorySize, 150 * 1024);
        if (e == hipSuccess)
            e = hipFuncSetAttribute((const void*)k_mlp_fwd_w<NK, NCT, WAVES, false>, hipFuncAttributeMaxDynamicSharedMemorySize, 2 * NF * 1024 + 2048 * 4);
        if (e != hipSuccess) {
            pk_set_error("pk_ln_mlp_wide_fwd: cannot raise the LDS limit: %s", hipGetErrorString(e));
            return (int)e;
        }
        attr_set = true;
    }
    const int need = (a.M + 32 * WAVES - 1) / (32 * WAVES);
    if (resident) {
        const int cus = pk_cu_count_block();
        hipLaunchKernelGGL((k_mlp_fwd_w<NK, NCT, WAVES, true>), dim3(need < cus ? need : cus), dim3(64 * WAVES), lds, st, a, C, c_real, HD);
    } else {
        hipLaunchKernelGGL((k_mlp_fwd_w<NK, NCT, WAVES, false>), dim3(need), dim3(64 * WAVES), lds, st, a, C, c_real, HD);
    }
    return pk_launch_status("pk_ln_mlp_wide_fwd");
}
extern "C" int pk_ln_mlp_wide_fwd(const void* x, const float* gamma, const float* beta, const void* w1, const float* b1, const void* w2,
                                  const float* b2, const float* row_scale, void* y, int M, int C, int c_real, int hidden,
                                  int rows_per_sample, float eps, void* stream) {
    PK_SUPPORTED(pk_ln_mlp_wide_supported(C, hidden, 0), "pk_ln_mlp_wide_fwd: C=%d hidden=%d (built for C = 80 / 128 / 160 / 256 / 320, hidden %% 32 == 0)", C, hidden);
    PK_REQUIRE(x && gamma && beta && w1 && b1 && w2 && b2 && y && M > 0, "pk_ln_mlp_wide_fwd: null pointer / bad size");
    PK_REQUIRE(c_real > 0 && c_real <= C, "pk_ln_mlp_wide_fwd: c_real=%d outside (0, C=%d]", c_real, C);
    PK_REQUIRE(!row_scale || rows_per_sample > 0, "pk_ln_mlp_wide_fwd: scale needs rows_per_sample");
    PK_REQUIRE((int64_t)M * C < 0x3fffffffLL && (int64_t)hidden * C < 0x1fffffffLL, "pk_ln_mlp_wide_fwd: tensor too large for 32-bit byte offsets");
    PK_REQUIRE(((((uintptr_t)x) | ((uintptr_t)y) | ((uintptr_t)w1) | ((uintptr_t)w2) | ((uintptr_t)gamma) | ((uintptr_t)beta) | ((uintptr_t)b2)) & 15) == 0,
               "pk_ln_mlp_wide_fwd: 16-byte alignment");
    MlpArgs a{};
    a.x = (const uint16_t*)x; a.out = (uint16_t*)y; a.gamma = gamma; a.beta = beta; a.b1 = b1; a.b2 = b2; a.scale = row_scale;
    a.w1 = (const uint16_t*)w1; a.w2 = (const uint16_t*)w2; a.M = M; a.rows_per_sample = rows_per_sample > 0 ? rows_per_sample : 1; a.eps = eps;
    hipStream_t st = (hipStream_t)stream;
    switch (C) {
        case 80: return mlp_wide_launch<3, 5, 8>(a, C, c_real, hidden, st);
        case 128: return mlp_wide_launch<4, 8, 8>(a, C, c_real, hidden, st);
        case 160: return mlp_wide_launch<5, 10, 8>(a, C, c_real, hidden, st);
        case 256: return mlp_wide_launch<8, 16, 4>(a, C, c_real, hidden, st);
        default: return mlp_wide_launch<10, 20, 4>(a, C, c_real, hidden, st);
    }
}

extern "C" int pk_ln_mlp_bwd_dx(const void* dy, const void* x, const float* gamma, const float* beta, const void* w1, const float* b1,
                                const void* w1_t, const void* w2_t, const float* row_scale, void* dx, float* ln_partial, int M, int C,
                                int rows_per_sample, float eps, void* stream) {
    MlpArgs a{};
    a.x = (const uint16_t*)x; a.dy = (const uint16_t*)dy; a.out = (uint16_t*)dx; a.gamma = gamma; a.beta = beta; a.b1 = b1; a.scale = row_scale;
    a.w1 = (const uint16_t*)w1; a.w1t = (const uint16_t*)w1_t; a.w2t = (const uint16_t*)w2_t; a.part = ln_partial;
    a.M = M; a.rows_per_sample = rows_per_sample > 0 ? rows_per_sample : 1; a.eps = eps;
    int rc = mlp_check("pk_ln_mlp_bwd_dx", a, C);
    if (rc) return rc;
    PK_REQUIRE(dy && w1 && w1_t && w2_t && dx && ln_partial, "pk_ln_mlp_bwd_dx: null pointer");
    const dim3 grid(pk_ln_mlp_dx_blocks(M, C)), block(256);
    if (C == 32) hipLaunchKernelGGL(k_mlp_bwd_dx<32>, grid, block, 0, (hipStream_t)stream, a);
    else hipLaunchKernelGGL(k_mlp_bwd_dx<64>, grid, block, 0, (hipStream_t)stream, a);
    return pk_launch_status("pk_ln_mlp_bwd_dx");
}

extern "C" int pk_ln_mlp_bwd_dw(const void* dy, const void* x, const float* gamma, const float* beta, const void* w1, const float* b1,
                                const void* w2_t, const float* row_scale, float* slabs, int M, int C, int rows_per_sample, float eps,
                                void* stream) {
    MlpArgs a{};
    a.x = (const uint16_t*)x; a.dy = (const uint16_t*)dy; a.gamma = gamma; a.beta = beta; a.b1 = b1; a.scale = row_scale;
    a.w1 = (const uint16_t*)w1; a.w2t = (const uint16_t*)w2_t; a.part = slabs;
    a.M = M; a.rows_per_sample = rows_per_sample > 0 ? rows_per_sample : 1; a.eps = eps;
    int rc = mlp_check("pk_ln_mlp_bwd_dw", a, C);
    if (rc) return rc;
    PK_REQUIRE(dy && w1 && w2_t && slabs, "pk_ln_mlp_bwd_dw: null pointer");
    const int hs = mlp_hidden_slice(C);
    const dim3 grid(pk_ln_mlp_dw_blocks(M, C), (4 * C) / hs), block(256);
    hipStream_t st = (hipStream_t)stream;
    if (C == 32) hipLaunchKernelGGL((k_mlp_bwd_dw<32, 64>), grid, block, 0, st, a);
    else hipLaunchKernelGGL((k_mlp_bwd_dw<64, 32>), grid, block, 0, st, a);
    return pk_launch_status("pk_ln_mlp_bwd_dw");
}
```

### infantposeestimation_gaussianbias_amd/csrc/pk_common.h

```cpp
#pragma once
#include <hip/hip_runtime.h>
#include <stdint.h>
#include <stdio.h>

#include "../../include/posekernels.h"


#define PK_WAVE 64

typedef __attribute__((ext_vector_type(8))) short bf16x8;
typedef __attribute__((ext_vector_type(4))) float f32x4;
typedef __attribute__((ext_vector_type(4))) unsigned int u32x4;
#define OOB_OFF 0x80000000u

void pk_set_error(const char* fmt, ...);

#define PK_REQUIRE(cond, ...)          \
    do {                               \
        if (!(cond)) {                 \
            pk_set_error(__VA_ARGS__); \
            return PK_ERR_INVALID;     \
        }                              \
    } while (0)

#define PK_SUPPORTED(cond, ...)        \
    do {                               \
        if (!(cond)) {                 \
            pk_set_error(__VA_ARGS__); \
            return PK_ERR_UNSUPPORTED; \
        }                              \
    } while (0)

static inline int pk_launch_status(const char* what) {
    hipError_t e = hipGetLastError();
    if (e != hipSuccess) {
        pk_set_error("%s: launch failed: %s", what, hipGetErrorString(e));
        return (int)e;
    }
    return PK_OK;
}

__device__ __forceinline__ float wave_sum(float v) {
#pragma unroll
    for (int o = 32; o > 0; o >>= 1) v += __shfl_xor(v, o, 64);
    return v;
}
__device__ __forceinline__ float wave_max(float v) {
#pragma unroll
    for (int o = 32; o > 0; o >>= 1) v = fmaxf(v, __shfl_xor(v, o, 64));
    return v;
}

__device__ __forceinline__ float block_sum(float v, float* red) {
    const int lane = threadIdx.x & 63, w = threadIdx.x >> 6, nw = (blockDim.x + 63) >> 6;
    v = wave_sum(v);
    __syncthreads();
    if (lane == 0) red[w] = v;
    __syncthreads();
    float t = 0.f;
    for (int i = 0; i < nw; ++i) t += red[i];
    return t;
}
__device__ __forceinline__ float block_max(float v, float* red) {
    const int lane = threadIdx.x & 63, w = threadIdx.x >> 6, nw = (blockDim.x + 63) >> 6;
    v = wave_max(v);
    __syncthreads();
    if (lane == 0) red[w] = v;
    __syncthreads();
    float t = red[0];
    for (int i = 1; i < nw; ++i) t = fmaxf(t, red[i]);
    return t;
}

__device__ __forceinline__ float bf16_to_f32(uint16_t h) { return __uint_as_float(((uint32_t)h) << 16); }
typedef __attribute__((ext_vector_type(2))) float pk_f32x2;
typedef __attribute__((ext_vector_type(2))) __bf16 pk_bf16x2;
__device__ __forceinline__ uint16_t f32_to_bf16(float f) { return __builtin_bit_cast(uint16_t, (__bf16)f); }
__device__ __forceinline__ uint32_t pack_bf16x2(float lo, float hi) {
    return __builtin_bit_cast(uint32_t, __builtin_convertvector((pk_f32x2){lo, hi}, pk_bf16x2));
}

typedef __attribute__((ext_vector_type(4))) float pk_f32x4;
struct GeluTerms { float hw, e; };
__device__ __forceinline__ GeluTerms gelu_terms(float x) {
    const float ax = fabsf(x);
    const float t = __builtin_amdgcn_rcpf(__fmaf_rn(0.3275911f * 0.70710678118654752440f, ax, 1.f));
    float q = __fmaf_rn(0.5f * 1.061405429f, t, 0.5f * -1.453152027f);
    q = __fmaf_rn(q, t, 0.5f * 1.421413741f);
    q = __fmaf_rn(q, t, 0.5f * -0.284496736f);
    q = __fmaf_rn(q, t, 0.5f * 0.254829592f);
    const float e = __builtin_amdgcn_exp2f((x * x) * (-0.5f * 1.44269504088896340736f));
    return GeluTerms{(q * t) * e, e};
}
__device__ __forceinline__ float gelu_erf(float x) {
    const GeluTerms g = gelu_terms(x);
    return __fmaf_rn(-fabsf(x), g.hw, fmaxf(x, 0.f));
}
__device__ __forceinline__ float gelu_cdf(float x, float hw) { return 0.5f + copysignf(0.5f - hw, x); }
__device__ __forceinline__ float gelu_grad(float x) {
    const GeluTerms g = gelu_terms(x);
    return __fmaf_rn(x * 0.39894228040143267794f, g.e, gelu_cdf(x, g.hw));
}
__device__ __forceinline__ void gelu_both(float x, float& val, float& grad) {
    const GeluTerms g = gelu_terms(x);
    val = __fmaf_rn(-fabsf(x), g.hw, fmaxf(x, 0.f));
    grad = __fmaf_rn(x * 0.39894228040143267794f, g.e, gelu_cdf(x, g.hw));
}
__device__ __forceinline__ pk_f32x4 gelu_erf(pk_f32x4 x) { return (pk_f32x4){gelu_erf(x[0]), gelu_erf(x[1]), gelu_erf(x[2]), gelu_erf(x[3])}; }
__device__ __forceinline__ pk_f32x4 gelu_grad(pk_f32x4 x) { return (pk_f32x4){gelu_grad(x[0]), gelu_grad(x[1]), gelu_grad(x[2]), gelu_grad(x[3])}; }
__device__ __forceinline__ void gelu_both(pk_f32x4 x, pk_f32x4& val, pk_f32x4& grad) {
#pragma unroll
    for (int i = 0; i < 4; ++i) {
        float a, b;
        gelu_both(x[i], a, b);
        val[i] = a;
        grad[i] = b;
    }
}
#define PK_GELU_CLAMP 4.2f
#define PK_GELU_C0 0.79781485f
#define PK_GELU_C1 -0.13272066f
#define PK_GELU_C2 0.019660205f
#define PK_GELU_C3 -0.0022282742f
#define PK_GELU_C4 0.0001891444f
#define PK_GELU_C5 -1.1521039e-05f
#define PK_GELU_C6 4.6870278e-07f
#define PK_GELU_C7 -1.1265554e-08f
#define PK_GELU_C8 1.1994644e-10f
__device__ __forceinline__ float erf_rsqrt2(float x) {
    const float xc = __builtin_amdgcn_fmed3f(x, -PK_GELU_CLAMP, PK_GELU_CLAMP);
    const float s = xc * xc;
    float q = __fmaf_rn(PK_GELU_C8, s, PK_GELU_C7);
    q = __fmaf_rn(q, s, PK_GELU_C6);
    q = __fmaf_rn(q, s, PK_GELU_C5);
    q = __fmaf_rn(q, s, PK_GELU_C4);
    q = __fmaf_rn(q, s, PK_GELU_C3);
    q = __fmaf_rn(q, s, PK_GELU_C2);
    q = __fmaf_rn(q, s, PK_GELU_C1);
    q = __fmaf_rn(q, s, PK_GELU_C0);
    return xc * q;
}
__device__ __forceinline__ pk_f32x4 erf_rsqrt2(pk_f32x4 x) {
    pk_f32x4 xc;
#pragma unroll
    for (int i = 0; i < 4; ++i) xc[i] = __builtin_amdgcn_fmed3f(x[i], -PK_GELU_CLAMP, PK_GELU_CLAMP);
    const pk_f32x4 s = xc * xc;
    pk_f32x4 q = __builtin_elementwise_fma((pk_f32x4)(PK_GELU_C8), s, (pk_f32x4)(PK_GELU_C7));
    q = __builtin_elementwise_fma(q, s, (pk_f32x4)(PK_GELU_C6));
    q = __builtin_elementwise_fma(q, s, (pk_f32x4)(PK_GELU_C5));
    q = __builtin_elementwise_fma(q, s, (pk_f32x4)(PK_GELU_C4));
    q = __builtin_elementwise_fma(q, s, (pk_f32x4)(PK_GELU_C3));
    q = __builtin_elementwise_fma(q, s, (pk_f32x4)(PK_GELU_C2));
    q = __builtin_elementwise_fma(q, s, (pk_f32x4)(PK_GELU_C1));
    q = __builtin_elementwise_fma(q, s, (pk_f32x4)(PK_GELU_C0));
    return xc * q;
}
__device__ __forceinline__ float gelu_erf_poly(float x) {
    const float h = 0.5f * x;
    return __fmaf_rn(h, erf_rsqrt2(x), h);
}
__device__ __forceinline__ pk_f32x4 gelu_erf_poly(pk_f32x4 x) {
    const pk_f32x4 h = x * 0.5f;
    return __builtin_elementwise_fma(h, erf_rsqrt2(x), h);
}
__device__ __forceinline__ float softplus_(float v) { return v > 20.f ? v : log1pf(__expf(v)); }

__device__ __forceinline__ float row16_sum(float v) {
#if defined(__HIP_DEVICE_COMPILE__)
    v += __int_as_float(__builtin_amdgcn_update_dpp(0, __float_as_int(v), 0xB1, 0xF, 0xF, true));
    v += __int_as_float(__builtin_amdgcn_update_dpp(0, __float_as_int(v), 0x4E, 0xF, 0xF, true));
    v += __int_as_float(__builtin_amdgcn_update_dpp(0, __float_as_int(v), 0x124, 0xF, 0xF, true));
    v += __int_as_float(__builtin_amdgcn_update_dpp(0, __float_as_int(v), 0x128, 0xF, 0xF, true));
#endif
    return v;
}


__device__ __forceinline__ float xor16_partner(float v) {
#if defined(__HIP_DEVICE_COMPILE__)
    return __int_as_float(__builtin_amdgcn_ds_swizzle(__float_as_int(v), 0x401F));
#else
    return v;
#endif
}
__device__ __forceinline__ float xor16_sum(float v) {
#if defined(__HIP_DEVICE_COMPILE__)
    return v + xor16_partner(v);
#else
    return v;
#endif
}
__device__ __forceinline__ float xor32_sum(float v) {
#if defined(__HIP_DEVICE_COMPILE__)
    const auto r = __builtin_amdgcn_permlane32_swap(__float_as_uint(v), __float_as_uint(v), false, false);
    return __uint_as_float(r[0]) + __uint_as_float(r[1]);
#else
    return v;
#endif
}
__device__ __forceinline__ float xor16_max(float v) {
#if defined(__HIP_DEVICE_COMPILE__)
    return fmaxf(v, xor16_partner(v));
#else
    return v;
#endif
}
__device__ __forceinline__ float xor32_max(float v) {
#if defined(__HIP_DEVICE_COMPILE__)
    const auto r = __builtin_amdgcn_permlane32_swap(__float_as_uint(v), __float_as_uint(v), false, false);
    return fmaxf(__uint_as_float(r[0]), __uint_as_float(r[1]));
#else
    return v;
#endif
}

template <int L>
__device__ __forceinline__ float lanes_sum(float v) {
#if defined(__HIP_DEVICE_COMPILE__)
    if (L >= 2) v += __int_as_float(__builtin_amdgcn_update_dpp(0, __float_as_int(v), 0xB1, 0xF, 0xF, true));
    if (L >= 4) v += __int_as_float(__builtin_amdgcn_update_dpp(0, __float_as_int(v), 0x4E, 0xF, 0xF, true));
    if (L >= 8) v += __int_as_float(__builtin_amdgcn_update_dpp(0, __float_as_int(v), 0x141, 0xF, 0xF, true));
    if (L >= 16) v += __int_as_float(__builtin_amdgcn_update_dpp(0, __float_as_int(v), 0x140, 0xF, 0xF, true));
    if (L >= 32) v = xor16_sum(v);
    if (L >= 64) v = xor32_sum(v);
#endif
    return v;
}
```

Baseline: 4220 images/sec.

## Skip DropPath-dropped samples in fused MLP and window-attention kernels

Result: no change. 4247 images/sec (median of 6 runs) (+0.6%).

```diff
diff --git a/infantposeestimation_gaussianbias_amd/csrc/pk_block.hip b/infantposeestimation_gaussianbias_amd/csrc/pk_block.hip
--- a/infantposeestimation_gaussianbias_amd/csrc/pk_block.hip
+++ b/infantposeestimation_gaussianbias_amd/csrc/pk_block.hip
@@ -112,12 +112,83 @@
     }
 }
 
-template <int C>
-__global__ void __launch_bounds__(256) k_mlp_fwd(MlpArgs p) {
+
+__device__ __forceinline__ bool mlp_group_dropped(const MlpArgs& p, int grp, int lane) {
+    const int row = grp * 32 + (lane & 31);
+    const bool live = row < p.M && p.scale[row / p.rows_per_sample] != 0.f;
+    return __ballot(live) == 0ull;
+}
+template <int C, typename Rsrc>
+__device__ __forceinline__ void mlp_copy_group(const Rsrc src, const Rsrc dst, int grp, int M, int lane) {
+    const int i16 = lane & 15, g = lane >> 4;
+#pragma unroll
+    for (int rt = 0; rt < 2; ++rt) {
+        const int row = grp * 32 + 16 * rt + i16;
+#pragma unroll
+        for (int k = 0; k < C / 32; ++k) {
+            const unsigned off = row < M ? (unsigned)row * (unsigned)(C * 2) + (32 * k + 8 * g) * 2 : OOB_OFF;
+            __builtin_amdgcn_raw_buffer_store_b128(__builtin_amdgcn_raw_buffer_load_b128(src, off, 0, 0), dst, off, 0, 0);
+        }
+    }
+}
+template <int C, typename Rsrc>
+__device__ __forceinline__ void attn_copy_window(const Rsrc src, const Rsrc dst, const int32_t* __restrict__ rowmap, int w, int lane) {
+    const int i16 = lane & 15, g = lane >> 4;
+#pragma unroll
+    for (int t = 0; t < 4; ++t) {
+        const int n = 16 * t + i16;
+        const int row = n < 49 ? rowmap[w * 49 + n] : -1;
+#pragma unroll
+        for (int k = 0; k < C / 32; ++k) {
+            const unsigned off = row >= 0 ? (unsigned)row * (unsigned)(C * 2) + (32 * k + 8 * g) * 2 : OOB_OFF;
+            __builtin_amdgcn_raw_buffer_store_b128(__builtin_amdgcn_raw_buffer_load_b128(src, off, 0, 0), dst, off, 0, 0);
+        }
+    }
+}
+__device__ __forceinline__ void zero_fill16(void* dst, int n16, int lane) {
+    for (int i = lane; i < n16; i += 64) reinterpret_cast<u32x4*>(dst)[i] = (u32x4){0u, 0u, 0u, 0u};
+}
+
+template <bool INPLACE, typename Unit, typename Copy, typename Dropped>
+__device__ __forceinline__ void drop_walk_run(const PkDropWalk& walk, const unsigned char* order, int first, int stride, Unit unit, Copy copy,
+                                              Dropped dropped_in_place) {
+    int c = first;
+    if (INPLACE) {
+        for (; c < walk.total; c += stride) {
+            if (walk.mode && dropped_in_place(c)) copy(c);
+            else unit(c);
+        }
+        return;
+    }
+    bool dropped;
+    auto lookup = [&](int ci) {
+        return walk.mode ? __builtin_amdgcn_readfirstlane(pk_drop_unit(min(ci, walk.total - 1), walk.ups, walk.kept_units, order, &dropped)) : ci;
+    };
+    int u = lookup(c);
+    for (; c < walk.kept_units; c += stride) {
+        const int u_next = lookup(c + stride);
+        unit(u);
+        u = u_next;
+    }
+    for (; c < walk.total; c += stride) {
+        const int u_next = lookup(c + stride);
+        copy(u);
+        u = u_next;
+    }
+}
+
+static inline bool mlp_compact(int M, int rows_per_sample) {
+    return pk_drop_compact((M + 31) / 32, rows_per_sample >> 5, (rows_per_sample & 31) == 0 && M % rows_per_sample == 0);
+}
+
+template <int C, bool INPLACE>
+__device__ __forceinline__ void mlp_fwd_body(const MlpArgs& p) {
     constexpr int HD = 4 * C, NK = C / 32, NT = HD / 16, NS = HD / 32, NCT = C / 16, RT = 2;
     __shared__ __attribute__((aligned(16))) u32x4 sW1[NT * NK * 64];
     __shared__ __attribute__((aligned(16))) u32x4 sW2[NCT * NS * 64];
     __shared__ __attribute__((aligned(16))) float sB1[HD];
+    __shared__ unsigned char sOrder[PK_DROP_CAP];
+    __shared__ int sCnt[4];
     const int tid = threadIdx.x, lane_ = tid & 63, wave = tid >> 6, i16 = lane_ & 15, g = lane_ >> 4;
     stage_frags(sW1, p.w1, NT * NK, C, [](int f, int i) { return hid(f / NK, i); }, [](int f) { return 32 * (f % NK); });
     stage_frags(sW2, p.w2, NCT * NS, HD, [](int f, int i) { return 16 * (f / NS) + i; }, [](int f) { return 32 * (f % NS); });
@@ -133,13 +204,14 @@
     f32x4 b2v[NCT];
 #pragma unroll
     for (int ct = 0; ct < NCT; ++ct) b2v[ct] = *reinterpret_cast<const f32x4*>(p.b2 + 16 * ct + 4 * g);
+    const int ngroups = (p.M + 16 * RT - 1) / (16 * RT);
+    const PkDropWalk walk = pk_drop_walk(p.scale, ngroups, p.rows_per_sample >> 5, !INPLACE, sOrder, sCnt);
     __syncthreads();
     const auto rx = MAKE_RSRC(p.x);
     const auto ro = MAKE_RSRC(p.out);
-    const int ngroups = (p.M + 16 * RT - 1) / (16 * RT);
     const float inv_c = 1.f / (float)C;
     const f32x4 zero = {0.f, 0.f, 0.f, 0.f};
-    for (int grp = blockIdx.x * 4 + wave; grp < ngroups; grp += gridDim.x * 4) {
+    auto unit = [&](const int grp) {
         const int lane = opaque_lane<C != 32>(lane_);
         u32x4 xr[RT][NK];
         u32x2 xo[RT][NCT];
@@ -202,8 +274,15 @@
                 const f32x4 o = (y[rt][ct] + b2v[ct]) * sc[rt] + unpack4(xo[rt][ct]);
                 __builtin_amdgcn_raw_buffer_store_b64(pack4(o), ro, rbase[rt] == OOB_OFF ? OOB_OFF : rbase[rt] + (16 * ct + 4 * g) * 2, 0, 0);
             }
-    }
-}
+    };
+    drop_walk_run<INPLACE>(walk, sOrder, blockIdx.x * 4 + __builtin_amdgcn_readfirstlane(wave), gridDim.x * 4, unit,
+                           [&](const int grp) { mlp_copy_group<C>(rx, ro, grp, p.M, lane_); },
+                           [&](const int grp) { return mlp_group_dropped(p, grp, lane_); });
+}
+template <int C>
+__global__ void __launch_bounds__(256) k_mlp_fwd(MlpArgs p) { mlp_fwd_body<C, false>(p); }
+template <int C>
+__global__ void __launch_bounds__(256) k_mlp_fwd_inplace(MlpArgs p) { mlp_fwd_body<C, true>(p); }
 
 template <int NK, int NCT, int WAVES, bool RESIDENT>
 __global__ void __launch_bounds__(64 * WAVES) k_mlp_fwd_w(MlpArgs p, int C, int c_real, int HD) {
@@ -377,14 +456,16 @@
     }
 }
 
-template <int C>
-__global__ void __launch_bounds__(256) k_mlp_bwd_dx(MlpArgs p) {
+template <int C, bool INPLACE>
+__device__ __forceinline__ void mlp_bwd_dx_body(const MlpArgs& p) {
     constexpr int HD = 4 * C, NK = C / 32, NT = HD / 16, NS = HD / 32, NCT = C / 16, RT = 2;
     __shared__ __attribute__((aligned(16))) u32x4 sW1[NT * NK * 64];
     __shared__ __attribute__((aligned(16))) u32x4 sW2T[NT * NK * 64];
     __shared__ __attribute__((aligned(16))) u32x4 sW1T[NCT * NS * 64];
     __shared__ __attribute__((aligned(16))) float sB1[HD];
     __shared__ float sRed[4][2][C];
+    __shared__ unsigned char sOrder[PK_DROP_CAP];
+    __shared__ int sCnt[4];
     const int tid = threadIdx.x, lane_ = tid & 63, wave = tid >> 6, i16 = lane_ & 15, g = lane_ >> 4;
     stage_frags(sW1, p.w1, NT * NK, C, [](int f, int i) { return hid(f / NK, i); }, [](int f) { return 32 * (f % NK); });
     stage_frags(sW2T, p.w2t, NT * NK, C, [](int f, int i) { return hid(f / NK, i); }, [](int f) { return 32 * (f % NK); });
@@ -405,13 +486,14 @@
         gamA[ct] = *reinterpret_cast<const f32x4*>(p.gamma + 16 * ct + 4 * g);
         dgam[ct] = dbet[ct] = zero;
     }
+    const int ngroups = (p.M + 16 * RT - 1) / (16 * RT);
+    const PkDropWalk walk = pk_drop_walk(p.scale, ngroups, p.rows_per_sample >> 5, !INPLACE, sOrder, sCnt);
     __syncthreads();
     const auto rx = MAKE_RSRC(p.x);
     const auto rg = MAKE_RSRC(p.dy);
     const auto ro = MAKE_RSRC(p.out);
-    const int ngroups = (p.M + 16 * RT - 1) / (16 * RT);
     const float inv_c = 1.f / (float)C;
-    for (int grp = blockIdx.x * 4 + wave; grp < ngroups; grp += gridDim.x * 4) {
+    auto unit = [&](const int grp) {
         const int lane = opaque_lane<true>(lane_);
         u32x4 xr[RT][NK], dyr[RT][NK];
         u32x2 xo[RT][NCT], dyo[RT][NCT];
@@ -510,7 +592,10 @@
                 __builtin_amdgcn_raw_buffer_store_b64(pack4(o), ro, rbase[rt] == OOB_OFF ? OOB_OFF : rbase[rt] + (16 * ct + 4 * g) * 2, 0, 0);
             }
         }
-    }
+    };
+    drop_walk_run<INPLACE>(walk, sOrder, blockIdx.x * 4 + __builtin_amdgcn_readfirstlane(wave), gridDim.x * 4, unit,
+                           [&](const int grp) { mlp_copy_group<C>(rg, ro, grp, p.M, lane_); },
+                           [&](const int grp) { return mlp_group_dropped(p, grp, lane_); });
 #pragma unroll
     for (int ct = 0; ct < NCT; ++ct)
 #pragma unroll
@@ -529,9 +614,13 @@
         p.part[(size_t)blockIdx.x * 2 * C + tid] = ((sRed[0][which][c] + sRed[1][which][c]) + sRed[2][which][c]) + sRed[3][which][c];
     }
 }
-
-template <int C, int HS>
-__global__ void __launch_bounds__(256) k_mlp_bwd_dw(MlpArgs p) {
+template <int C>
+__global__ void __launch_bounds__(256) k_mlp_bwd_dx(MlpArgs p) { mlp_bwd_dx_body<C, false>(p); }
+template <int C>
+__global__ void __launch_bounds__(256) k_mlp_bwd_dx_inplace(MlpArgs p) { mlp_bwd_dx_body<C, true>(p); }
+
+template <int C, int HS, bool INPLACE>
+__device__ __forceinline__ void mlp_bwd_dw_body(const MlpArgs& p) {
     constexpr int NK = C / 32, NTS = HS / 16, NSP = HS / 32, NCT = C / 16, RT = 2;
     constexpr int PV = C + 8, PH = 40;
     constexpr int TILE_HALFS = 2 * 32 * PV + 2 * 32 * PH;
@@ -541,6 +630,8 @@
     __shared__ __attribute__((aligned(16))) u32x4 sW2T[NTS * NK * 64];
     __shared__ __attribute__((aligned(16))) float sB1[HS];
     __shared__ __attribute__((aligned(16))) unsigned char sScratch[SCRATCH_BYTES];
+    __shared__ unsigned char sOrder[PK_DROP_CAP];
+    __shared__ int sCnt[4];
     const int tid = threadIdx.x, lane_ = tid & 63, wave = tid >> 6, i16 = lane_ & 15, g = lane_ >> 4;
     const int h0 = blockIdx.y * HS;
     stage_frags(sW1, p.w1 + (size_t)h0 * C, NTS * NK, C, [](int f, int i) { return 16 * (f / NK) + i; }, [](int f) { return 32 * (f % NK); });
@@ -569,12 +660,13 @@
     }
 #pragma unroll
     for (int ct = 0; ct < NCT; ++ct) db2[ct] = 0.f;
+    const int ngroups = (p.M + 16 * RT - 1) / (16 * RT);
+    const PkDropWalk walk = pk_drop_walk(p.scale, ngroups, p.rows_per_sample >> 5, !INPLACE, sOrder, sCnt);
     __syncthreads();
     const auto rx = MAKE_RSRC(p.x);
     const auto rg = MAKE_RSRC(p.dy);
-    const int ngroups = (p.M + 16 * RT - 1) / (16 * RT);
     const float inv_c = 1.f / (float)C;
-    for (int grp = blockIdx.x * 4 + wave; grp < ngroups; grp += gridDim.x * 4) {
+    auto unit = [&](const int grp) {
         const int lane = opaque_lane<true>(lane_);
         u32x4 xr[RT][NK], dyr[RT][NK];
         float sc[RT];
@@ -654,7 +746,9 @@
             }
             LDS_FENCE();
         }
-    }
+    };
+    drop_walk_run<INPLACE>(walk, sOrder, blockIdx.x * 4 + __builtin_amdgcn_readfirstlane(wave), gridDim.x * 4, unit, [](const int) {},
+                           [&](const int grp) { return mlp_group_dropped(p, grp, lane_); });
     float* slab = reinterpret_cast<float*>(sScratch);
 #pragma unroll 1
     for (int w = 0; w < 4; ++w) {
@@ -695,6 +789,10 @@
     float* dst = p.part + ((size_t)blockIdx.y * gridDim.x + blockIdx.x) * SLAB;
     for (int i = tid * 4; i < SLAB; i += 1024) *reinterpret_cast<f32x4*>(dst + i) = *reinterpret_cast<const f32x4*>(slab + i);
 }
+template <int C, int HS>
+__global__ void __launch_bounds__(256) k_mlp_bwd_dw(MlpArgs p) { mlp_bwd_dw_body<C, HS, false>(p); }
+template <int C, int HS>
+__global__ void __launch_bounds__(256) k_mlp_bwd_dw_inplace(MlpArgs p) { mlp_bwd_dw_body<C, HS, true>(p); }
 
 struct AttnArgs {
     const uint16_t* x;
@@ -715,13 +813,15 @@
 #define AT_N 49
 __device__ __forceinline__ int rel_a7(int t) { return 13 * (t / 7) + t % 7; }
 
-template <int C>
-__global__ void __launch_bounds__(256) k_attn_fwd(AttnArgs p) {
+template <int C, bool INPLACE>
+__device__ __forceinline__ void attn_fwd_body(const AttnArgs& p) {
     constexpr int HEADS = C / 32, NK = C / 32, NCT = C / 16;
     __shared__ __attribute__((aligned(16))) u32x4 sWqkv[HEADS * 6 * NK * 64];
     __shared__ __attribute__((aligned(16))) u32x4 sWp[NCT * HEADS * 64];
     __shared__ __attribute__((aligned(16))) float sBqkv[3 * C];
     __shared__ float sBias[HEADS][176];
+    __shared__ unsigned char sOrder[PK_DROP_CAP];
+    __shared__ int sCnt[4];
     const int tid = threadIdx.x, lane_ = tid & 63, wave = tid >> 6, g_ = lane_ >> 4;
     stage_frags(sWqkv, p.wqkv, HEADS * 6 * NK, C,
                 [](int f, int i) {
@@ -752,12 +852,19 @@
             const int j = 16 * cj + 4 * g_ + r;
             aj[cj][r] = j < AT_N ? 84 - rel_a7(j) : -1;
         }
+    const PkDropWalk walk = pk_drop_walk(p.scale, p.n_windows, p.windows_per_sample, !INPLACE, sOrder, sCnt);
     __syncthreads();
     const auto rx = MAKE_RSRC(p.x);
     const auto ro = MAKE_RSRC(p.out);
     const float inv_c = 1.f / (float)C;
     const f32x4 zero = {0.f, 0.f, 0.f, 0.f};
-    for (int w = blockIdx.x * 4 + wave; w < p.n_windows; w += gridDim.x * 4) {
+    auto copy = [&](const int w) {
+        attn_copy_window<C>(rx, ro, p.rowmap, w, lane_);
+        if (p.o_save) zero_fill16(p.o_save + (size_t)w * AT_N * C, AT_N * C / 8, lane_);
+        if (p.lse)
+            for (int i = lane_; i < HEADS * AT_N; i += 64) p.lse[(size_t)w * HEADS * AT_N + i] = 0.f;
+    };
+    auto unit = [&](const int w) {
         const int lane = opaque_lane<true>(lane_), i16 = lane & 15, g = lane >> 4;
         int row[4];
         u32x4 xr[4][NK];
@@ -892,8 +999,14 @@
                 const f32x4 v = (accY[t][ct] + bpv[ct]) * sc + unpack4(xo[t][ct]);
                 __builtin_amdgcn_raw_buffer_store_b64(pack4(v), ro, row[t] >= 0 ? (unsigned)row[t] * (unsigned)(C * 2) + (16 * ct + 4 * g) * 2 : OOB_OFF, 0, 0);
             }
-    }
-}
+    };
+    drop_walk_run<INPLACE>(walk, sOrder, blockIdx.x * 4 + __builtin_amdgcn_readfirstlane(wave), gridDim.x * 4, unit, copy,
+                           [&](const int w) { return p.scale[w / p.windows_per_sample] == 0.f; });
+}
+template <int C>
+__global__ void __launch_bounds__(256) k_attn_fwd(AttnArgs p) { attn_fwd_body<C, false>(p); }
+template <int C>
+__global__ void __launch_bounds__(256) k_attn_fwd_inplace(AttnArgs p) { attn_fwd_body<C, true>(p); }
 
 template <int NK, int NCT, int HEADS, int WAVES>
 __global__ void __launch_bounds__(64 * WAVES) k_attn_fwd_w(AttnArgs p, int C, int c_real) {
@@ -1137,8 +1250,8 @@
     }
 }
 
-template <int C>
-__global__ void __launch_bounds__(256, 2) k_attn_bwd(AttnArgs p, float* __restrict__ part_ln, float* __restrict__ part_rpb) {
+template <int C, bool INPLACE>
+__device__ __forceinline__ void attn_bwd_body(const AttnArgs& p, float* __restrict__ part_ln, float* __restrict__ part_rpb) {
     constexpr int HEADS = C / 32, NK = C / 32, NCT = C / 16, NKQ = 3 * C / 32;
     constexpr int F_A = 6 * NK, F_B = 4 * NK;
     __shared__ __attribute__((aligned(16))) u32x4 sWa[HEADS * F_A * 64];
@@ -1158,6 +1271,8 @@
     __shared__ float sFoldBuf[FOLD_PAD + 4 * AT_N * AT_N + FOLD_PAD];
     float* const sFold0 = sFoldBuf + FOLD_PAD;
     __shared__ float sRed[4][2][C];
+    __shared__ unsigned char sOrder[PK_DROP_CAP];
+    __shared__ int sCnt[4];
     const int tid = threadIdx.x, lane_ = tid & 63, wave = tid >> 6;
     stage_frags(sWa, p.wqkv, HEADS * F_A, C,
                 [](int f, int i) { const int r = f / NK, et = r & 1, part = (r >> 1) % 3, h = r / 6; return part * C + 32 * h + 16 * et + i; },
@@ -1182,13 +1297,19 @@
     f32x4 dgam[NCT], dbet[NCT];
 #pragma unroll
     for (int ct = 0; ct < NCT; ++ct) dgam[ct] = dbet[ct] = zero;
+    const PkDropWalk walk = pk_drop_walk(p.scale, p.n_windows, p.windows_per_sample, !INPLACE, sOrder, sCnt);
     __syncthreads();
     const auto rx = MAKE_RSRC(p.x);
     const auto rg = MAKE_RSRC(p.dy);
     const auto ro = MAKE_RSRC(p.out);
     const auto rs = MAKE_RSRC(p.o_save);
     const float inv_c = 1.f / (float)C, scale = p.softmax_scale, scale2 = p.softmax_scale * LOG2E_F, inv_scale = 1.f / p.softmax_scale;
-    for (int w = blockIdx.x * 4 + wave; w < p.n_windows; w += gridDim.x * 4) {
+    auto copy = [&](const int w) {
+        attn_copy_window<C>(rg, ro, p.rowmap, w, lane_);
+        zero_fill16(p.dqkv + (size_t)w * AT_N * 3 * C, AT_N * 3 * C / 8, lane_);
+        zero_fill16(p.u_save + (size_t)w * AT_N * C, AT_N * C / 8, lane_);
+    };
+    auto unit = [&](const int w) {
         const int lane = opaque_lane<true>(lane_), i16 = lane & 15, g = lane >> 4;
         int row[4];
         f32x4 du[4][NCT];
@@ -1488,7 +1609,9 @@
                 __builtin_amdgcn_raw_buffer_store_b64(pack4(o), ro, valid ? (unsigned)rw * (unsigned)(C * 2) + (16 * ct + 4 * g) * 2 : OOB_OFF, 0, 0);
             }
         }
-    }
+    };
+    drop_walk_run<INPLACE>(walk, sOrder, blockIdx.x * 4 + __builtin_amdgcn_readfirstlane(wave), gridDim.x * 4, unit, copy,
+                           [&](const int w) { return p.scale[w / p.windows_per_sample] == 0.f; });
     const int i16 = lane_ & 15, g = lane_ >> 4;
 #pragma unroll
     for (int ct = 0; ct < NCT; ++ct)
@@ -1512,6 +1635,10 @@
         part_ln[(size_t)blockIdx.x * 2 * C + tid] = ((sRed[0][which][c] + sRed[1][which][c]) + sRed[2][which][c]) + sRed[3][which][c];
     }
 }
+template <int C>
+__global__ void __launch_bounds__(256, 2) k_attn_bwd(AttnArgs p, float* part_ln, float* part_rpb) { attn_bwd_body<C, false>(p, part_ln, part_rpb); }
+template <int C>
+__global__ void __launch_bounds__(256, 2) k_attn_bwd_inplace(AttnArgs p, float* part_ln, float* part_rpb) { attn_bwd_body<C, true>(p, part_ln, part_rpb); }
 
 static inline int attn_blocks(int n_windows) {
     constexpr int cap = 256;
@@ -1538,7 +1665,10 @@
     a.dqkv = (uint16_t*)dqkv; a.u_save = (uint16_t*)u_out; a.n_windows = n_windows;
     a.windows_per_sample = windows_per_sample > 0 ? windows_per_sample : 1; a.eps = eps; a.softmax_scale = 1.f / sqrtf(32.f);
     const dim3 grid(attn_blocks(n_windows)), block(256);
-    if (C == 32) hipLaunchKernelGGL(k_attn_bwd<32>, grid, block, 0, (hipStream_t)stream, a, ln_partial, rpb_partial);
+    if (a.scale && !pk_drop_compact(n_windows, a.windows_per_sample, true)) {
+        if (C == 32) hipLaunchKernelGGL(k_attn_bwd_inplace<32>, grid, block, 0, (hipStream_t)stream, a, ln_partial, rpb_partial);
+        else hipLaunchKernelGGL(k_attn_bwd_inplace<64>, grid, block, 0, (hipStream_t)stream, a, ln_partial, rpb_partial);
+    } else if (C == 32) hipLaunchKernelGGL(k_attn_bwd<32>, grid, block, 0, (hipStream_t)stream, a, ln_partial, rpb_partial);
     else hipLaunchKernelGGL(k_attn_bwd<64>, grid, block, 0, (hipStream_t)stream, a, ln_partial, rpb_partial);
     return pk_launch_status("pk_attn_block_bwd");
 }
@@ -1559,7 +1689,10 @@
     a.lse = lse; a.n_windows = n_windows; a.windows_per_sample = windows_per_sample > 0 ? windows_per_sample : 1; a.eps = eps;
     a.softmax_scale = 1.f / sqrtf(32.f);
     const dim3 grid(attn_blocks(n_windows)), block(256);
-    if (C == 32) hipLaunchKernelGGL(k_attn_fwd<32>, grid, block, 0, (hipStream_t)stream, a);
+    if (a.scale && !pk_drop_compact(n_windows, a.windows_per_sample, true)) {
+        if (C == 32) hipLaunchKernelGGL(k_attn_fwd_inplace<32>, grid, block, 0, (hipStream_t)stream, a);
+        else hipLaunchKernelGGL(k_attn_fwd_inplace<64>, grid, block, 0, (hipStream_t)stream, a);
+    } else if (C == 32) hipLaunchKernelGGL(k_attn_fwd<32>, grid, block, 0, (hipStream_t)stream, a);
     else hipLaunchKernelGGL(k_attn_fwd<64>, grid, block, 0, (hipStream_t)stream, a);
     return pk_launch_status("pk_attn_block_fwd");
 }
@@ -1644,7 +1777,10 @@
     if (rc) return rc;
     PK_REQUIRE(w1 && w2 && b2 && y, "pk_ln_mlp_fwd: null pointer");
     const dim3 grid(mlp_blocks(M, MLP_FWD_WGS)), block(256);
-    if (C == 32) hipLaunchKernelGGL(k_mlp_fwd<32>, grid, block, 0, (hipStream_t)stream, a);
+    if (a.scale && !mlp_compact(M, a.rows_per_sample)) {
+        if (C == 32) hipLaunchKernelGGL(k_mlp_fwd_inplace<32>, grid, block, 0, (hipStream_t)stream, a);
+        else hipLaunchKernelGGL(k_mlp_fwd_inplace<64>, grid, block, 0, (hipStream_t)stream, a);
+    } else if (C == 32) hipLaunchKernelGGL(k_mlp_fwd<32>, grid, block, 0, (hipStream_t)stream, a);
     else hipLaunchKernelGGL(k_mlp_fwd<64>, grid, block, 0, (hipStream_t)stream, a);
     return pk_launch_status("pk_ln_mlp_fwd");
 }
@@ -1724,7 +1860,10 @@
     if (rc) return rc;
     PK_REQUIRE(dy && w1 && w1_t && w2_t && dx && ln_partial, "pk_ln_mlp_bwd_dx: null pointer");
     const dim3 grid(pk_ln_mlp_dx_blocks(M, C)), block(256);
-    if (C == 32) hipLaunchKernelGGL(k_mlp_bwd_dx<32>, grid, block, 0, (hipStream_t)stream, a);
+    if (a.scale && !mlp_compact(M, a.rows_per_sample)) {
+        if (C == 32) hipLaunchKernelGGL(k_mlp_bwd_dx_inplace<32>, grid, block, 0, (hipStream_t)stream, a);
+        else hipLaunchKernelGGL(k_mlp_bwd_dx_inplace<64>, grid, block, 0, (hipStream_t)stream, a);
+    } else if (C == 32) hipLaunchKernelGGL(k_mlp_bwd_dx<32>, grid, block, 0, (hipStream_t)stream, a);
     else hipLaunchKernelGGL(k_mlp_bwd_dx<64>, grid, block, 0, (hipStream_t)stream, a);
     return pk_launch_status("pk_ln_mlp_bwd_dx");
 }
@@ -1742,7 +1881,10 @@
     const int hs = mlp_hidden_slice(C);
     const dim3 grid(pk_ln_mlp_dw_blocks(M, C), (4 * C) / hs), block(256);
     hipStream_t st = (hipStream_t)stream;
-    if (C == 32) hipLaunchKernelGGL((k_mlp_bwd_dw<32, 64>), grid, block, 0, st, a);
+    if (a.scale && !mlp_compact(M, a.rows_per_sample)) {
+        if (C == 32) hipLaunchKernelGGL((k_mlp_bwd_dw_inplace<32, 64>), grid, block, 0, st, a);
+        else hipLaunchKernelGGL((k_mlp_bwd_dw_inplace<64, 32>), grid, block, 0, st, a);
+    } else if (C == 32) hipLaunchKernelGGL((k_mlp_bwd_dw<32, 64>), grid, block, 0, st, a);
     else hipLaunchKernelGGL((k_mlp_bwd_dw<64, 32>), grid, block, 0, st, a);
     return pk_launch_status("pk_ln_mlp_bwd_dw");
 }
diff --git a/infantposeestimation_gaussianbias_amd/csrc/pk_common.h b/infantposeestimation_gaussianbias_amd/csrc/pk_common.h
--- a/infantposeestimation_gaussianbias_amd/csrc/pk_common.h
+++ b/infantposeestimation_gaussianbias_amd/csrc/pk_common.h
@@ -70,6 +70,65 @@
     float t = red[0];
     for (int i = 1; i < nw; ++i) t = fmaxf(t, red[i]);
     return t;
+}
+
+#define PK_DROP_CAP 256
+struct PkDropWalk {
+    int mode;
+    int ups;
+    int kept_units;
+    int total;
+};
+__host__ __device__ inline int pk_drop_unit(int c, int ups, int kept_units, const unsigned char* order, bool* dropped) {
+    const int s = c / ups;
+    *dropped = c >= kept_units;
+    return (int)order[s] * ups + (c - s * ups);
+}
+__host__ __device__ inline int pk_drop_order(const float* scale, int B, unsigned char* order) {
+    int n = 0;
+    for (int s = 0; s < B; ++s)
+        if (scale[s] != 0.f) order[n++] = (unsigned char)s;
+    const int kept = n;
+    for (int s = 0; s < B; ++s)
+        if (!(scale[s] != 0.f)) order[n++] = (unsigned char)s;
+    return kept;
+}
+__host__ __device__ inline bool pk_drop_compact(int n_units, int ups, bool aligned) {
+    if (!aligned || ups <= 0 || n_units % ups != 0) return false;
+    return n_units / ups <= PK_DROP_CAP;
+}
+__device__ __forceinline__ PkDropWalk pk_drop_walk(const float* __restrict__ scale, int n_units, int ups, bool compact, unsigned char* order, int* cnt) {
+    PkDropWalk w{0, ups, n_units, n_units};
+    if (!scale) return w;
+    w.mode = 1;
+    if (!compact) return w;
+    const int B = n_units / ups;
+    const int lane = threadIdx.x & 63, wave = threadIdx.x >> 6;
+    const unsigned long long below = (1ull << lane) - 1ull;
+    int n_kept;
+    if (B <= 64) {
+        const bool in = lane < B, kept = in && scale[in ? lane : 0] != 0.f;
+        const unsigned long long km = __ballot(kept), dm = __ballot(in && !kept);
+        n_kept = __popcll(km);
+        if (wave == 0 && in) order[kept ? __popcll(km & below) : n_kept + __popcll(dm & below)] = (unsigned char)lane;
+    } else {
+        const int s = threadIdx.x;
+        const bool in = s < B, kept = in && scale[in ? s : 0] != 0.f;
+        const unsigned long long km = __ballot(kept), dm = __ballot(in && !kept);
+        if (lane == 0) cnt[wave] = __popcll(km);
+        __syncthreads();
+        int before = 0;
+        n_kept = 0;
+        for (int i = 0; i < 4; ++i) {
+            const int c = cnt[i];
+            n_kept += c;
+            if (i < wave) before += c;
+        }
+        if (in) order[kept ? before + __popcll(km & below) : n_kept + (64 * wave - before) + __popcll(dm & below)] = (unsigned char)s;
+    }
+    w.mode = 2;
+    w.kept_units = __builtin_amdgcn_readfirstlane(n_kept) * ups;
+    return w;
 }
 
 __device__ __forceinline__ float bf16_to_f32(uint16_t h) { return __uint_as_float(((uint32_t)h) << 16); }
```
